# mbortolon97/6dgs

Hardware: AMD Instinct MI355X
Metric: poses/sec (higher is better)
Workload: dtype f32

## Files before the change

### 6dgs_amd/_lib.py

```python
from __future__ import annotations

import ctypes as C
import os

_HERE = os.path.dirname(os.path.abspath(__file__))
LIB_PATH = os.path.join(_HERE, "csrc", "lib6dgs_hip.so")
if os.environ.get("SIXDGS_LIB"):
    LIB_PATH = os.path.abspath(os.environ["SIXDGS_LIB"])

vp = C.c_void_p
i64 = C.c_int64
i32 = C.c_int
sz = C.c_size_t


PROFILE_SLOTS = 128
ABI_VERSION = 10


class Profile(C.Structure):
    _fields_ = [("count", i32), ("start", vp * PROFILE_SLOTS), ("stop", vp * PROFILE_SLOTS),
                ("flops", C.c_double * PROFILE_SLOTS), ("bytes", C.c_double * PROFILE_SLOTS)]


# ... 5 lines not shown
    "sixdgs_abi_version": (i32, []),
    "sixdgs_error_string": (C.c_char_p, [i32]),
    "sixdgs_mask_degraded": (i32, [vp, i64, i32, vp, vp]),
    "sixdgs_sym_eig_3x3": (i32, [vp, i64, vp, vp, vp]),
    "sixdgs_normals_knn": (i32, [vp, i64, vp, i64, i32, vp, vp, vp]),
    "sixdgs_normals_knn_grid_workspace_bytes": (sz, [i64]),
    "sixdgs_normals_knn_grid": (i32, [vp, i64, vp, i64, i32, vp, vp, vp, sz, vp]),
    "sixdgs_emit_quadricell_count": (i32, [vp, vp, i32, vp, vp, i64, vp, i32, i32, vp, vp, vp, vp]),
    "sixdgs_emit_quadricell_write": (i32, [vp, vp, i32, vp, vp, vp, i32, i32, vp, i64, vp, i32, i32, vp, vp, vp, vp, vp, vp]),
    "sixdgs_quadricell_cell_counts": (i32, [vp, i64, i32, vp, vp, vp, vp]),
    "sixdgs_quadricell_centers": (i32, [vp, i64, i32, i32, vp, vp, vp, vp]),
    "sixdgs_isocell_distribution": (i32, [i32, i32, vp, C.POINTER(i64), vp]),
    "sixdgs_rotate_isocell": (i32, [vp, i64, vp, i64, vp, vp]),
    "sixdgs_emit_isocell": (i32, [vp, vp, i32, vp, vp, vp, i32, i32, vp, i64, vp, vp, i64, vp, vp, vp, vp, vp]),
    "sixdgs_eval_sh_color": (i32, [vp, i32, vp, i64, i32, vp, vp]),
    "sixdgs_splat_views_workspace_bytes": (sz, [i64, i32, i32, i32]),
    "sixdgs_splat_views": (i32, [vp, vp, i32, vp, vp, i32, i32, i64, vp, i32, i32, i32, i32, C.c_float, C.c_float, vp, vp, vp, vp, sz, vp]),
    "sixdgs_raster_views_workspace_bytes": (sz, [i64, i32, i32, i32, i64]),
    "sixdgs_raster_views": (i32, [vp, vp, i32, vp, vp, i32, vp, vp, i32, i32, i64, vp, i32, i32, i32, C.c_float, vp, vp, vp, i32, vp, i64, vp, vp, sz,
                                  vp, C.POINTER(Profile)]),
    "sixdgs_raster_views_backward_workspace_bytes": (sz, [i64, i32, i32, i32, i64]),
    "sixdgs_raster_views_backward": (i32, [vp, vp, i32, vp, vp, i32, vp, vp, i32, i32, i64, vp, i32, i32, i32, C.c_float, vp, vp, i64, vp, sz,
                                           vp, vp, vp, vp, vp, vp, vp, vp, sz, vp, C.POINTER(Profile)]),
    "sixdgs_photometric_loss_workspace_bytes": (sz, [i32, i32, i32, i32]),
    "sixdgs_photometric_loss": (i32, [vp, i32, vp, i32, i32, i32, i32, i32, C.c_float, vp, vp, vp, vp, vp, sz, vp, C.POINTER(Profile)]),
    "sixdgs_pose_compose": (i32, [vp, vp, i32, vp, vp]),
    "sixdgs_pose_step": (i32, [vp, vp, vp, vp, i64, i32, i32, i32, C.c_float, C.c_float, C.c_float, C.c_float] + [vp] * 10 + [vp]),
    "sixdgs_refine_poses_workspace_bytes": (sz, [i64, i32, i32, i32, i64]),
    "sixdgs_refine_poses": (i32, [vp, vp, i32, vp, vp, i32, vp, vp, i32, i32, i64, vp, i32, i32, i32, C.c_float, vp, vp, i32, i32, C.c_float,
                                  i32, C.c_float, C.c_float, C.c_float, C.c_float, i64] + [vp] * 7 + [vp, sz, vp]),
    "sixdgs_target_pyramid": (i32, [vp, i32, i32, i32, i32, i32, vp, i32, vp, vp, vp]),
    "sixdgs_pose_rebase": (i32, [vp, vp, i32, vp, vp]),
    "sixdgs_refine_poses_levels_workspace_bytes": (sz, [i64, i32, i32, vp, vp, vp]),
    "sixdgs_refine_poses_levels": (i32, [vp, vp, i32, vp, vp, i32, vp, vp, i32, i32, i64, vp, i32, C.c_float, vp, C.c_float, i32] + [vp] * 7
                                   + [C.c_float, C.c_float, C.c_float] + [vp] * 8 + [vp, sz, vp]),
    "sixdgs_gaussian_adam": (i32, [i64, i32, i32] + [vp] * 6 + [vp] * 6 + [vp, vp, vp, C.c_float, C.c_float, C.c_float, vp, i64, vp, vp]),
    "sixdgs_opacity_reset": (i32, [vp, i64, i32, vp, vp, C.c_float, vp]),
    "sixdgs_fit_scene_workspace_bytes": (sz, [i64, i32, i32, i32, i32, i64]),
    "sixdgs_fit_scene": (i32, [vp, vp, i32, vp, vp, i32, vp, vp, i32, i64, vp, i32, i32, i32, C.c_float, vp, vp, i32, i32, C.c_float, i32, i32,
                               vp, vp, vp, vp, i32, C.c_float, C.c_float, C.c_float, C.c_float, i64] + [vp] * 5 + [vp, sz, vp]),
    "sixdgs_densify_stats": (i32, [i64, i32, i32, i32, i64, vp, sz, vp, sz, vp, vp, vp, vp, vp, vp, vp]),
    "sixdgs_densify_workspace_bytes": (sz, [i64]),
    "sixdgs_densify": (i32, [i64, i32] + [vp] * 6 + [i32, i32] + [vp] * 6 + [C.c_float] * 4 + [i32, i32, i64] + [vp] * 8 + [vp, vp, vp, sz, vp]),
    "sixdgs_knn_workspace_bytes": (sz, [i64]),
    "sixdgs_knn_mean_dist2": (i32, [i64, vp, vp, vp, sz, vp]),
    "sixdgs_fit_scene_steps_workspace_bytes": (sz, [i64, i32, i32, i32, i32, i64]),
    "sixdgs_fit_scene_steps": (i32, [vp, vp, i32, vp, vp, i32, vp, vp, i32, i64, vp, i32, i32, i32, C.c_float, vp, vp, i32, i32, C.c_float, i32, i32,
                                     vp, vp, vp, vp, vp, vp, i32, i32, C.c_float, C.c_float, C.c_float, C.c_float, i64] + [vp] * 5 + [vp] * 3
                               + [vp, sz, vp]),
    "sixdgs_packed_weights_floats": (sz, []),
    "sixdgs_pack_weights": (i32, [vp] * 13 + [C.POINTER(ScorerWeights), vp]),
    "sixdgs_ray_encode": (i32, [vp, vp, vp, i64, vp, vp]),
    "sixdgs_ray_keys_workspace_bytes": (sz, [i64, i64]),
    "sixdgs_ray_keys": (i32, [vp, vp, vp, i64, C.POINTER(ScorerWeights), vp, vp, vp, sz, vp]),
    "sixdgs_ray_keys_ex": (i32, [vp, vp, vp, i64, C.POINTER(ScorerWeights), vp, vp, vp, vp, vp, vp, sz, vp, C.POINTER(Profile), i32]),
    "sixdgs_key_planes_f16_bytes": (sz, [i64]),
    "sixdgs_split_planes_f16": (i32, [vp, i64, i64, vp, vp, vp]),
    "sixdgs_score_pass1": (i32, [vp, vp, vp, i32, vp, vp, vp, i64, i32, vp, vp, sz, vp, C.POINTER(Profile), i32]),
    "sixdgs_score_pass2": (i32, [vp, vp, i32, i32, i64, i32, vp, vp, vp, vp, sz, vp, i32]),
    "sixdgs_score_backward_workspace_bytes": (sz, [i32]),
    "sixdgs_score_backward": (i32, [vp, vp, i32, vp, i64, vp, vp, vp, vp, vp, sz, vp]),
    "sixdgs_score_backward_split_workspace_bytes": (sz, [i32, i64, i32]),
    "sixdgs_score_backward_split": (i32, [vp, vp, i32, vp, i64, vp, vp, vp, vp, i32, vp, sz, vp]),
    "sixdgs_score_topk_ex": (i32, [vp, vp, vp, i32, vp, vp, vp, i64, i32, vp, vp, vp, vp, vp, sz, vp, C.POINTER(Profile), i32]),
    "sixdgs_score_select_workspace_bytes": (sz, [i64, i32, i32, i32]),
    "sixdgs_score_select": (i32, [vp, vp, vp, i32, vp, vp, vp, i64, vp, vp, i64, i32, i32, vp, vp, vp, vp, sz, vp, C.POINTER(Profile)]),
    "sixdgs_tok_attention": (i32, [vp, i64, i32, i32, i32, vp, i64, vp]),
    "sixdgs_im2col": (i32, [vp, i64, i64, i64, i64, i32, i32, i32, i32, i32, i32, vp, vp]),
    "sixdgs_u8_to_planar": (i32, [vp, i32, i64, vp, vp, vp]),
    "sixdgs_image_prep": (i32, [vp, i32, i32, i32, vp, i32, i32, i32, i32, i32, vp, vp, vp, vp]),
    "sixdgs_tok_pack_bytes": (sz, [i32, i32]),
    "sixdgs_tok_pack": (i32, [vp, i32, i32, i64, vp, vp, vp]),
    "sixdgs_tok_linear": (i32, [vp, i64, i32, i64, i32, vp, vp, C.c_float, vp, vp, vp, i32, i32, vp, i64, vp, vp, i64, vp]),
    "sixdgs_key_planes_norm_max": (i32, [vp, vp, i64, vp, vp]),
    "sixdgs_select_workspace_bytes": (sz, [i64, i32, i32, i32]),
    "sixdgs_select_candidates_workspace_bytes": (sz, [i64, i32, i32, i32]),
    "sixdgs_select_begin": (i32, [vp, vp, vp, i32, vp, vp, i64, i64, vp, vp, vp, sz, vp]),
    "sixdgs_select_sweep_plan": (i32, [vp, i32, vp, vp, i32]),
    "sixdgs_select_sweep": (i32, [vp, vp, vp, i32, vp, vp, i64, vp, vp, vp, i64, vp, vp, sz, vp, C.POINTER(Profile)]),
    "sixdgs_select_candidates": (i32, [vp, i64, i64, vp, vp, vp, i32, vp, vp, vp, i32, i32, vp, vp, vp, sz, vp]),
    "sixdgs_select_rescore": (i32, [vp, vp, i32, vp, vp, i32, vp, vp, vp, vp, i64, i32, i32, i32, vp, vp, vp, vp, sz, vp]),
    "sixdgs_select_sample_stats": (i32, [vp, vp, vp, i32, vp, vp, i64, vp, vp, sz, vp]),
    "sixdgs_select_prepare": (i32, [vp, vp, i32, i64, i64, vp, vp, vp]),
    "sixdgs_select_topk_u": (i32, [vp, i64, i64, vp, i32, i32, vp, vp, sz, vp]),
    "sixdgs_linear_splitk_workspace_bytes": (sz, [i64, i32, i32]),
    "sixdgs_linear_splitk": (i32, [vp, i64, i32, i64, vp, i64, vp, i32, i32, vp, i64, i32, vp, sz, vp, i32]),
    "sixdgs_linear_ex": (i32, [vp, i64, i32, i64, vp, i64, vp, i32, i32, vp, i64, vp, i32]),
    "sixdgs_profile_collect": (i32, [C.POINTER(Profile), C.POINTER(C.c_double), C.POINTER(C.c_double), C.POINTER(C.c_double),
                                    C.POINTER(i32)]),
    "sixdgs_linear": (i32, [vp, i64, i32, i64, vp, i64, vp, i32, i32, vp, i64, vp]),
    "sixdgs_q_proj": (i32, [vp, vp, i32, C.POINTER(ScorerWeights), vp, vp]),
    "sixdgs_score_topk_workspace_bytes": (sz, [i64, i32, i32]),
    "sixdgs_score_topk_workspace_bytes_ex": (sz, [i64, i32, i32, i32, i32]),
    "sixdgs_score_topk": (i32, [vp, vp, i32, vp, i64, i32, vp, vp, vp, vp, vp, sz, vp]),
    "sixdgs_topk_workspace_bytes": (sz, [i64, i32, i32]),
    "sixdgs_topk": (i32, [vp, i64, i32, i32, vp, vp, vp, sz, vp]),
    "sixdgs_distance_target_workspace_bytes": (sz, [i64]),
    "sixdgs_distance_target": (i32, [vp, vp, i64, vp, i32, vp, vp, vp, sz, vp]),
    "sixdgs_solve_pose": (i32, [vp, vp, i64, vp, vp, i32, vp, vp, i32, vp, vp, vp, vp, vp, vp, vp]),
    "sixdgs_solve_pose_consensus_workspace_bytes": (sz, [i32, i32]),
    "sixdgs_solve_pose_consensus": (i32, [vp, vp, i64, vp, vp, i32, vp, vp, i32, C.c_float, i32] + [vp] * 10 + [vp, sz, vp]),
}

_lib = None


def load():
    global _lib
    if _lib is not None:
        return _lib
    import torch

    if not os.path.exists(LIB_PATH):
        raise RuntimeError(
            f"6dgs_amd: {LIB_PATH} is missing -- build it with `python -m 6dgs_amd.build` / __graft_entry__.build(); "
            "there is no CPU fallback for the product path")
    try:
        lib = C.CDLL(LIB_PATH)
    except OSError as e:
        raise RuntimeError(f"6dgs_amd: cannot load {LIB_PATH}: {e}") from e
    for name, (res, args) in SIGNATURES.items():
        try:
            fn = getattr(lib, name)
        except AttributeError as e:
            raise RuntimeError(f"6dgs_amd: {LIB_PATH} does not export {name}") from e
        fn.restype = res
        fn.argtypes = args
    if lib.sixdgs_abi_version() != ABI_VERSION:
        raise RuntimeError(f"6dgs_amd: ABI version mismatch (library {lib.sixdgs_abi_version()}, binding {ABI_VERSION})")
    _lib = lib
    return lib


def check(status: int, what: str = ""):
    if status != 0:
        msg = load().sixdgs_error_string(int(status)).decode()
        raise RuntimeError(f"6dgs_amd: {what or 'call'} failed: {msg} (status {status})")
```

### 6dgs_amd/build.py

```python
from __future__ import annotations

import os
import subprocess
import sys

HERE = os.path.dirname(os.path.abspath(__file__))
CSRC = os.path.join(HERE, "csrc")
LIB = os.path.join(CSRC, "lib6dgs_hip.so")
HOSTCHECK = os.path.join(CSRC, "libsixdgs_hostcheck.so")
SOURCES = ["geometry.hip", "gemm.hip", "dense.hip", "score.hip", "score_bwd.hip", "pose.hip", "pose_consensus.hip", "vit.hip", "splat.hip", "raster.hip", "photometric.hip", "refine.hip", "fit.hip", "densify.hip", "knn.hip", "pyramid.hip"]
HEADERS = ["common.h", "device_math.h", "gemm_kernel.h", "dense.h", os.path.join("..", "..", "include", "sixdgs.h"), "dense_layout.h", "sweep_plan.h", "sweep_layout.h", "pose_step.h", "adam_step.h", "render_pass.h", "densify_rules.h", "knn_rules.h", "pyramid_rules.h"]
HIPCC = os.environ.get("HIPCC", "/opt/rocm/bin/hipcc")
FLAGS = ["--offload-arch=gfx950", "-O3", "-std=c++17", "-fPIC", "-ffp-contract=off", "-Wall", "-Wno-unused-function"]
FLAGS += os.environ.get("SIXDGS_EXTRA_FLAGS", "").split()


def _stale(target, deps):
    if not os.path.exists(target):
        return True
    t = os.path.getmtime(target)
    return any(os.path.getmtime(d) > t for d in deps)


def build(force: bool = False, verbose: bool = False) -> str:
    deps = [os.path.join(CSRC, s) for s in SOURCES + HEADERS]
    if force or _stale(LIB, deps):
        objs = []
        procs = []
        for s in SOURCES:
            o = os.path.join(CSRC, s.replace(".hip", ".o"))
            objs.append(o)
            cmd = [HIPCC, *FLAGS, "-c", os.path.join(CSRC, s), "-o", o]
            if verbose:
                print(" ".join(cmd))
            procs.append((cmd, subprocess.Popen(cmd, stdout=subprocess.PIPE, stderr=subprocess.STDOUT, text=True)))
        for cmd, p in procs:
            out, _ = p.communicate()
            if p.returncode != 0:
                sys.stderr.write(out)
                raise RuntimeError("hipcc failed: " + " ".join(cmd))
            if verbose and out.strip():
                print(out)
        cmd = [HIPCC, "--offload-arch=gfx950", "-shared", "-fPIC", *objs, "-o", LIB]
        subprocess.check_call(cmd)
    return LIB


def build_hostcheck(force: bool = False) -> str:
    src = os.path.join(CSRC, "hostcheck.cpp")
    deps = [src, os.path.join(CSRC, "device_math.h"), os.path.join(CSRC, "dense_layout.h"), os.path.join(CSRC, "sweep_plan.h"),
            os.path.join(CSRC, "sweep_layout.h"), os.path.join(CSRC, "pose_step.h"), os.path.join(CSRC, "adam_step.h"), os.path.join(CSRC, "densify_rules.h"),
            os.path.join(CSRC, "knn_rules.h"), os.path.join(CSRC, "pyramid_rules.h")]
    if force or _stale(HOSTCHECK, deps):
        cmd = [HIPCC, "-x", "hip", "--offload-arch=gfx950", "-O2", "-std=c++17", "-fPIC", "-ffp-contract=off", "-shared", src,
               "-o", HOSTCHECK]
        subprocess.check_call(cmd)
    return HOSTCHECK


if __name__ == "__main__":
    print(build(force="--force" in sys.argv, verbose=True))
    print(build_hostcheck(force="--force" in sys.argv))
```

### 6dgs_amd/csrc/hostcheck.cpp

```cpp
#include <stdlib.h>

#include "device_math.h"
#include "sweep_plan.h"
#include "dense_layout.h"
#include "sweep_layout.h"
#include "pose_step.h"
#include "adam_step.h"
#include "densify_rules.h"
#include "knn_rules.h"
#include "pyramid_rules.h"

#include <algorithm>
#include <vector>
using namespace sdg;

extern "C" {

void hc_mask_degraded(const float* scale, long long n, int P, unsigned char* mask) {
  for (long long i = 0; i < n; ++i) {
    float side;
    mask[i] = total_rings(scale[3 * i], scale[3 * i + 1], scale[3 * i + 2], (float)P, &side) < (long long)P;
  }
}

long long hc_quadricell_centers(const float* scale, long long E, int P, int res, float* points, long long* eid) {
  long long C = 0;
  float* table = (float*)malloc(sizeof(float) * res);
  for (long long e = 0; e < E; ++e) {
    float a = scale[3 * e], b = scale[3 * e + 1], c = scale[3 * e + 2], side;
    long long rings = total_rings(a, b, c, (float)P, &side);
    for (long long ring = 0; ring < rings; ++ring) {
      Ring rg = ring_params(a, b, c, side, (float)rings, (float)ring);
      int npts = ring_cells(rg);
      if (!npts) continue;
      if (points) {
        double acc = 0.0;
        table[0] = 0.f;
        for (int j = 0; j < res - 1; ++j) { acc += (double)ring_table_increment(rg, j); table[j + 1] = (float)acc; }
        float last = table[res - 1];
        for (int j = 0; j < res; ++j) table[j] = kTwoPi * (table[j] / last);
        for (int j = 0; j < npts; ++j) {
          int pick = ring_table_pick(table, res, (float)j * rg.dtheta);
          V3 p = ring_point(rg, table[pick]);
          points[3 * (C + j)] = p.x; points[3 * (C + j) + 1] = p.y; points[3 * (C + j) + 2] = p.z;
          eid[C + j] = e;
        }
      }
      C += npts;
    }
  }
  free(table);
  return C;
}

long long hc_emit_rays(const float* points, const long long* eid, long long C, const float* normals, const float* centers,
                       const float* rot4, float* ori, float* dir, long long* mid) {
  long long r = 0;
  for (long long i = 0; i < C; ++i) {
    long long e = eid[i];
    float R[9];
    quat_to_rotmat(rot4 + 4 * e, R);
    V3 pw = rotate(R, v3(points[3 * i], points[3 * i + 1], points[3 * i + 2]));
    if (!hemisphere_keep(normals[3 * e], pw)) continue;
    V3 d = normalize_eps(pw);
    ori[3 * r] = pw.x + centers[3 * e]; ori[3 * r + 1] = pw.y + centers[3 * e + 1]; ori[3 * r + 2] = pw.z + centers[3 * e + 2];
    dir[3 * r] = d.x; dir[3 * r + 1] = d.y; dir[3 * r + 2] = d.z;
    mid[r++] = e;
  }
  return r;
}

void hc_sym_eig(const float* mats, long long n, float* vals, float* vecs) {
  for (long long i = 0; i < n; ++i) sym_eig_3x3(mats + 9 * i, vals + 3 * i, vecs ? vecs + 9 * i : nullptr);
}

void hc_normals_from_knn(const float* cloud, const long long* knn, long long nq, int k, float* normals) {
  float* nb = (float*)malloc(sizeof(float) * 3 * k);
  for (long long q = 0; q < nq; ++q) {
    for (int j = 0; j < k; ++j)
      for (int c = 0; c < 3; ++c) nb[3 * j + c] = cloud[3 * knn[q * k + j] + c];
    V3 n = normal_from_neighbours(nb, k);
    normals[3 * q] = n.x; normals[3 * q + 1] = n.y; normals[3 * q + 2] = n.z;
  }
  free(nb);
}

long long hc_isocell_dirs(int target, int n0, float* dirs) {
  int n = isocell_rings(target, n0);
// ... 167 lines not shown
void hc_knn_pair_d2(long long n, const float* q, const float* p, float* out) {
  for (long long i = 0; i < n; ++i) out[i] = kn::pair_d2(q[3 * i], q[3 * i + 1], q[3 * i + 2], p[3 * i], p[3 * i + 1], p[3 * i + 2]);
}
int hc_knn_boxed(long long n, const float* xyz, int box, float* mean_d2, int* visited) {
  if (n < 4 || box < 1) return -1;
  float lo[3], hi[3];
  for (int a = 0; a < 3; ++a) lo[a] = INFINITY, hi[a] = -INFINITY;
  for (long long i = 0; i < n; ++i)
    for (int a = 0; a < 3; ++a) {
      lo[a] = fminf(lo[a], xyz[3 * i + a]);
      hi[a] = fmaxf(hi[a], xyz[3 * i + a]);
    }
  std::vector<unsigned> code(n);
  std::vector<long long> order(n);
  for (long long i = 0; i < n; ++i) {
    code[i] = kn::morton(xyz + 3 * i, lo, hi);
    order[i] = i;
  }
  std::stable_sort(order.begin(), order.end(), [&](long long a, long long b) { return code[a] < code[b]; });
  const long long nb = (n + box - 1) / box;
  std::vector<float> s(3 * n), blo(3 * nb, INFINITY), bhi(3 * nb, -INFINITY);
  for (long long k = 0; k < n; ++k)
    for (int a = 0; a < 3; ++a) {
      const float c = s[3 * k + a] = xyz[3 * order[k] + a];
      blo[3 * (k / box) + a] = fminf(blo[3 * (k / box) + a], c);
      bhi[3 * (k / box) + a] = fmaxf(bhi[3 * (k / box) + a], c);
    }
  for (long long k = 0; k < n; ++k) {
    const float qx = s[3 * k], qy = s[3 * k + 1], qz = s[3 * k + 2];
    float b0 = INFINITY, b1 = INFINITY, b2 = INFINITY;
    const long long own = k / box;
    int walked = 0;
    for (long long step = 0; step < nb; ++step)
      for (int side = 0; side < (step ? 2 : 1); ++side) {
        const long long c = side ? own + step : own - step;
        if (c < 0 || c >= nb) continue;
        if (step && kn::box_d2(qx, qy, qz, &blo[3 * c], &bhi[3 * c]) >= b2) continue;
        ++walked;
        const long long end = std::min(n, (c + 1) * box);
        for (long long j = c * box; j < end; ++j)
          if (j != k) kn::insert3(kn::pair_d2(qx, qy, qz, s[3 * j], s[3 * j + 1], s[3 * j + 2]), b0, b1, b2);
      }
    mean_d2[order[k]] = kn::mean3(b0, b1, b2);
    if (visited) visited[order[k]] = walked;
  }
  return 0;
}
int hc_pyr_max_levels() { return pyr::kMaxLevels; }
int hc_pyr_max_downscale() { return pyr::kMaxDownscale; }
void hc_pyr_geometry(int W, int H, int d, const float* k4, int* geo4, float* k_out4) {
  const pyr::Level g = pyr::level_geometry(W, H, d);
  geo4[0] = g.w; geo4[1] = g.h; geo4[2] = g.ox; geo4[3] = g.oy;
  pyr::level_intrinsics(k4, d, g.ox, g.oy, k_out4);
}
int hc_pyr_target(const unsigned char* images, int views, int H, int W, int C, int composite, const float* background, int d, float* out) {
  if (d < 1 || d > pyr::kMaxDownscale || (C != 3 && C != 4) || (composite && C != 4)) return -1;
  const pyr::Level g = pyr::level_geometry(W, H, d);
  if (g.w < 1 || g.h < 1) return -1;
  float bg255[3] = {0.f, 0.f, 0.f};
  if (composite)
    for (int c = 0; c < 3; ++c) bg255[c] = pyr::background_term(background[c]);
  for (int v = 0; v < views; ++v)
    for (int y = 0; y < g.h; ++y)
      for (int x = 0; x < g.w; ++x)
        for (int c = 0; c < 3; ++c) {
          unsigned S = 0u, S2 = 0u;
          for (int j = 0; j < d; ++j)
            for (int i = 0; i < d; ++i) {
              const unsigned char* q = images + (((size_t)v * H + (size_t)(g.oy + y * d + j)) * W + (size_t)(g.ox + x * d + i)) * C;
              if (composite) {
                S += (unsigned)q[c] * (unsigned)q[3];
                S2 += 255u - (unsigned)q[3];
              } else {
                S += (unsigned)q[c];
              }
            }
          out[(((size_t)v * g.h + y) * g.w + x) * 3 + c] = composite ? pyr::value_composite(S, S2, bg255[c], d) : pyr::value_plain(S, d);
        }
  return 0;
}
void hc_pyr_keep_input(const float* best_loss_last, const float* loss_input, long long n, int* keep) {
  for (long long i = 0; i < n; ++i) keep[i] = pyr::keep_input(best_loss_last[i], loss_input[i]) ? 1 : 0;
}
int hc_dl_const(int which) {
  const int v[] = {dl::kSlabB, dl::kPRow, dl::kGran, dl::kGranSlab, dl::kChunkRun};
  return which >= 0 && which < 5 ? v[which] : -1;
}

}
```

### 6dgs_amd/csrc/score.hip

```cpp
#include <stdlib.h>

#include <cstdlib>
#include <cstdio>
#include "gemm_kernel.h"
#include "sweep_plan.h"
#include "sweep_layout.h"

using namespace sdg;

namespace {

constexpr int kT = SIXDGS_MAX_TOKENS;
constexpr float kSqrtD = 19.595917942265423f;

struct LogitsArgs {
  const float* q;
  const int* n_tok;
  const float* key;
  float* logits;
  float* partial;
  int64_t r, ldl;
  int tiles_per_group, n_tiles, n_groups;
  int b0;
};

template <int MMA>
__global__ void __launch_bounds__(256, 2) k_logits(LogitsArgs A) {
  __shared__ __attribute__((aligned(16))) char smem[TileSmem<MMA>::kBytes];
  __shared__ float part[2][128][2];
  const int bl = blockIdx.y;
  const int b = A.b0 + bl;
  const unsigned w = xcd_remap(blockIdx.x, gridDim.x);
  const int grp = (int)(w >> 1), m_tile = (int)(w & 1u);
  const int M = A.n_tok[b];
  const int row0 = m_tile * 128;
  float* pout = A.partial + (((int64_t)bl * A.n_groups + grp) * kT + row0) * 2;
  const int tid = threadIdx.x, lane = tid & 63, wave = tid >> 6;
  const int wm = wave >> 1, wn = wave & 1;
  float m_run = -INFINITY, s_run = 0.f;
  if (row0 < M) {
    GemmOperands g = {A.q + (int64_t)b * kT * SIXDGS_D, nullptr, A.key, SIXDGS_D, 0, SIXDGS_D, M, A.r, SIXDGS_D, SIXDGS_D};
    float* lg = A.logits + (int64_t)bl * kT * A.ldl;
    const int t_begin = grp * A.tiles_per_group;
    const int t_end = min(t_begin + A.tiles_per_group, A.n_tiles);
    for (int tile = t_begin; tile < t_end; ++tile) {
      const int64_t col0 = (int64_t)tile * kBN;
      f32x16 acc[2][2];
      gemm_tile<MMA>(g, row0, col0, smem, acc);
      const int64_t c0 = col0 + acc_col(wn, 0, lane), c1 = col0 + acc_col(wn, 1, lane);
      const bool v0 = c0 < A.r, v1 = c1 < A.r;
#pragma unroll
      for (int tm = 0; tm < 2; ++tm)
#pragma unroll
        for (int r = 0; r < 16; ++r) {
          const int row = row0 + acc_row(wm, tm, r, lane);
          const float l0 = acc[tm][0][r] / kSqrtD, l1 = acc[tm][1][r] / kSqrtD;
          if (row < M) {
            if (v0) lg[(int64_t)row * A.ldl + c0] = l0;
            if (v1) lg[(int64_t)row * A.ldl + c1] = l1;
          }
          float mx = fmaxf(v0 ? l0 : -INFINITY, v1 ? l1 : -INFINITY);
#pragma unroll
          for (int o = 16; o > 0; o >>= 1) mx = fmaxf(mx, __shfl_xor(mx, o, 64));
          float sm = 0.f;
          if (mx > -INFINITY) sm = (v0 ? expf(l0 - mx) : 0.f) + (v1 ? expf(l1 - mx) : 0.f);
#pragma unroll
          for (int o = 16; o > 0; o >>= 1) sm += __shfl_xor(sm, o, 64);
          if ((lane & 31) == 0) {
            const int lr = acc_row(wm, tm, r, lane);
            part[wn][lr][0] = mx;
            part[wn][lr][1] = sm;
          }
        }
      __syncthreads();
      if (tid < 128) {
#pragma unroll
        for (int h = 0; h < 2; ++h) {
          const float mt = part[h][tid][0], st = part[h][tid][1];
          if (mt > -INFINITY) {
            const float mn = fmaxf(m_run, mt);
            s_run = s_run * expf(m_run - mn) + st * expf(mt - mn);
            m_run = mn;
          }
        }
      }
    }
  }
  if (tid < 128) {
    pout[2 * tid] = m_run;
// ... 688 lines not shown
          if (!ragged) {
#pragma unroll
            for (int tn = 0; tn < 4; ++tn)
#pragma unroll
              for (int r = 0; r < 16; ++r) sum[r & 3] += __expf(acc[tm][tn][r] - mn);
          } else {
            int ray0 = wn * 128 + 4 * (lane >> 5);
            asm volatile("" : "+v"(ray0));
#pragma unroll
            for (int tn = 0; tn < 4; ++tn)
#pragma unroll
              for (int r = 0; r < 16; ++r)
                sum[r & 3] += (ray0 + tn * 32 + 8 * (r >> 2) + (r & 3) <= lim_cur) ? __expf(acc[tm][tn][r] - mn) : 0.f;
          }
          s_run[tm] = s_run[tm] * __expf(m_run[tm] - mn) + ((sum[0] + sum[1]) + (sum[2] + sum[3]));
          m_run[tm] = mn;
        }
      }
      kcur = knext;
      lim_cur = lim_next;
    }
    if constexpr (PIPE) {
      if (active) {
#pragma unroll
        for (int rb = 4; rb < sw::kRayBlocks; ++rb) {
#pragma unroll
          for (int k = 0; k < 8; ++k) sweep_epi_exp(E, acc16, zs16, ct16, lane_p, wn, rb, k >> 2, k & 3);
          sweep_epi_fold_a(E, lane_p);
          sweep_epi_fold_b(E, lane_p, rb);
          sweep_epi_fold_c(E, lane_p, rb);
        }
        sweep_epi_store(E, lane_p, 1);
      }
    }
    asm volatile("s_waitcnt vmcnt(0)" ::: "memory");
  }
  __syncthreads();
  float(*part)[256][2] = reinterpret_cast<float(*)[256][2]>(lds);
  if (S16) {
    int lm = lane;
    if (PERS) asm volatile("" : "+v"(lm));
#pragma unroll
    for (int tb = 0; tb < sw::kTokBlocks; ++tb) {
      float z = zs16[tb];
      z += __builtin_bit_cast(float, __builtin_amdgcn_ds_swizzle(__builtin_bit_cast(int, z), 0x401F));
      if (sw::part_writes(lm)) {
        float* pp = part[sw::part_row(wn, lm)][wm * 64 + sw::acc_token(lm, tb)];
        pp[0] = 0.f;
        pp[1] = z;
      }
    }
  } else {
#pragma unroll
  for (int tm = 0; tm < 2; ++tm) {
    float* pp = part[wn * 2 + (lane >> 5)][wm * 64 + tm * 32 + (lane & 31)];
    if (OUT == kOutUB) {
      pp[0] = 0.f;
      pp[1] = (zs[tm][0].x + zs[tm][0].y) + (zs[tm][1].x + zs[tm][1].y);
    } else {
      pp[0] = m_run[tm];
      pp[1] = s_run[tm];
    }
  }
  }
  __syncthreads();
  if (tid < 256) {
    float m = -INFINITY, sres = 0.f;
#pragma unroll
    for (int h = 0; h < 4; ++h) {
      const float mt = part[h][tid][0], st2 = part[h][tid][1];
      if (mt > -INFINITY) {
        const float mn = fmaxf(m, mt);
        sres = sres * __expf(m - mn) + st2 * __expf(mt - mn);
        m = mn;
      }
    }
    pout[2 * tid] = m;
    pout[2 * tid + 1] = sres;
  }
  if (PERS) __syncthreads();
  } while (PERS && (grp += A.n_sets) < A.n_groups);
}

__global__ void __launch_bounds__(256) k_split_tiles_f16(const float* __restrict__ src, int64_t rows, int64_t ld, char* __restrict__ dst,
                                                         float* __restrict__ inv_scale) {
  __shared__ float wmax[4];
  const int64_t row0 = (int64_t)blockIdx.x * 128;
  const int n = (int)min((int64_t)128, rows - row0);
  const float* base = src + row0 * ld;
  float m = 0.f;
  for (int i = threadIdx.x; i < n * 96; i += 256) {
    const int row = i / 96;
    const float4 v = *reinterpret_cast<const float4*>(base + (int64_t)row * ld + (i - row * 96) * 4);
    m = fmaxf(m, fmaxf(fmaxf(fabsf(v.x), fabsf(v.y)), fmaxf(fabsf(v.z), fabsf(v.w))));
  }
  m = sdg_wave_max(m);
  if (sdg_lane() == 0) wmax[sdg_wave()] = m;
  __syncthreads();
  m = fmaxf(fmaxf(wmax[0], wmax[1]), fmaxf(wmax[2], wmax[3]));
  int sh = 0;
  if (m > 0.f && m < INFINITY) {
    int e;
    frexpf(m, &e);
    sh = 14 - e;
    sh = sh > 100 ? 100 : (sh < -100 ? -100 : sh);
  }
  const float sc = ldexpf(1.f, sh);
  if (threadIdx.x == 0) inv_scale[blockIdx.x] = ldexpf(1.f, -sh);
  for (int i = threadIdx.x; i < n * 48; i += 256) {
    const int row = i / 48, k8 = i - row * 48;
    const float* sp = base + (int64_t)row * ld + k8 * 8;
    const float4 lo = *reinterpret_cast<const float4*>(sp);
    const float4 hi = *reinterpret_cast<const float4*>(sp + 4);
    const float x[8] = {lo.x * sc, lo.y * sc, lo.z * sc, lo.w * sc, hi.x * sc, hi.y * sc, hi.z * sc, hi.w * sc};
    f16x8 h, l;
#pragma unroll
    for (int e = 0; e < 8; ++e) {
      const _Float16 hh = (_Float16)x[e];
      h[e] = hh;
      l[e] = (_Float16)(x[e] - (float)hh);
    }
    char* d = dst + (row0 + row) * kRowF + (k8 >> 2) * kSlabF + (k8 & 3) * 16;
    *reinterpret_cast<f16x8*>(d) = h;
    *reinterpret_cast<f16x8*>(d + 64) = l;
  }
}

__global__ void __launch_bounds__(256) k_split_q_tiles_f16(const float* __restrict__ q, const int* __restrict__ n_tok, char* __restrict__ dst,
                                                           float* __restrict__ inv_scale) {
  __shared__ float wmax[4];
  const int bl = blockIdx.x >> 1, half = blockIdx.x & 1;
  const int n = min(128, max(0, n_tok[bl] - 128 * half));
  const float* base = q + ((int64_t)bl * kT + 128 * half) * SIXDGS_D;
  float m = 0.f;
  for (int i = threadIdx.x; i < n * 96; i += 256) {
    const float4 v = *reinterpret_cast<const float4*>(base + (int64_t)i * 4);
    m = fmaxf(m, fmaxf(fmaxf(fabsf(v.x), fabsf(v.y)), fmaxf(fabsf(v.z), fabsf(v.w))));
  }
  m = sdg_wave_max(m);
  if (sdg_lane() == 0) wmax[sdg_wave()] = m;
  __syncthreads();
  m = fmaxf(fmaxf(wmax[0], wmax[1]), fmaxf(wmax[2], wmax[3]));
  int sh = 0;
  if (m > 0.f && m < INFINITY) {
    int e;
    frexpf(m, &e);
    sh = 14 - e;
    sh = sh > 100 ? 100 : (sh < -100 ? -100 : sh);
  }
  const float sc = ldexpf(1.f, sh);
  if (threadIdx.x == 0) inv_scale[blockIdx.x] = ldexpf(1.f, -sh);
  char* const drow = dst + ((int64_t)bl * kT + 128 * half) * kRowF;
  for (int i = threadIdx.x; i < 128 * 48; i += 256) {
    const int row = i / 48, k8 = i - row * 48;
    f16x8 h, l;
    if (row < n) {
      const float* sp = base + (int64_t)row * SIXDGS_D + k8 * 8;
      const float4 lo = *reinterpret_cast<const float4*>(sp);
      const float4 hi = *reinterpret_cast<const float4*>(sp + 4);
      const float x[8] = {lo.x * sc, lo.y * sc, lo.z * sc, lo.w * sc, hi.x * sc, hi.y * sc, hi.z * sc, hi.w * sc};
#pragma unroll
      for (int e = 0; e < 8; ++e) {
        const _Float16 hh = (_Float16)x[e];
        h[e] = hh;
        l[e] = (_Float16)(x[e] - (float)hh);
      }
// ... 266 lines not shown
      if (w2 < wv) { og += sc[0][w2]; oe += sc[1][w2]; }
      tg += sc[0][w2];
      te += sc[1][w2];
    }
    __syncthreads();
    if (WRITE) {
      const unsigned long long below = (1ull << lane) - 1ull;
      if (gt) {
        const unsigned pos = base_g + run_g + og + __popcll(bg & below);
        if (pos < (unsigned)topk) { cand_key[(int64_t)b * topk + pos] = key; cand_idx[(int64_t)b * topk + pos] = i; }
      } else if (eq) {
        const unsigned re = base_e + run_e + oe + __popcll(be & below);
        if (re < st.remain) {
          const unsigned pos = n_greater + re;
          if (pos < (unsigned)topk) { cand_key[(int64_t)b * topk + pos] = key; cand_idx[(int64_t)b * topk + pos] = i; }
        }
      }
    }
    run_g += tg;
    run_e += te;
  }
  if (!WRITE && threadIdx.x == 0) {
    counts[((int64_t)b * gridDim.x + blockIdx.x) * 2] = run_g;
    counts[((int64_t)b * gridDim.x + blockIdx.x) * 2 + 1] = run_e;
  }
}

__global__ void __launch_bounds__(1024) k_topk_scan(const unsigned* __restrict__ counts, int nb, unsigned* __restrict__ offs, const int* __restrict__ only) {
  __shared__ unsigned sm[17];
  const int b = blockIdx.x;
  if (only != nullptr && only[b] == 0) return;
  for (int comp = 0; comp < 2; ++comp) {
    unsigned base = 0;
    for (int c0 = 0; c0 < nb; c0 += 1024) {
      const int i = c0 + threadIdx.x;
      const unsigned v = i < nb ? counts[((int64_t)b * nb + i) * 2 + comp] : 0u;
      unsigned tot;
      const unsigned ex = sdg_block_exclusive_scan<unsigned, 16>(v, sm, &tot);
      if (i < nb) offs[((int64_t)b * nb + i) * 2 + comp] = base + ex;
      base += tot;
    }
  }
}

__global__ void __launch_bounds__(1024) k_topk_sort(const unsigned* __restrict__ cand_key, const int64_t* __restrict__ cand_idx,
                                                     int topk, int k_eff, int64_t* __restrict__ idx, float* __restrict__ val, const int* __restrict__ only) {
  __shared__ unsigned sk[1024];
  __shared__ long long si[1024];
  const int b = blockIdx.x, t = threadIdx.x;
  if (only != nullptr && only[b] == 0) return;
  if (t < k_eff) { sk[t] = cand_key[(int64_t)b * topk + t]; si[t] = cand_idx[(int64_t)b * topk + t]; }
  else { sk[t] = 0u; si[t] = 0x7fffffffffffffffll; }
  __syncthreads();
  for (int size = 2; size <= 1024; size <<= 1)
    for (int strd = size >> 1; strd > 0; strd >>= 1) {
      const int p = t ^ strd;
      if (p > t) {
        const bool up = (t & size) == 0;
        const unsigned ka = sk[t], kb = sk[p];
        const long long ia = si[t], ib = si[p];
        const bool a_first = ka > kb || (ka == kb && ia < ib);
        if (up ? !a_first : a_first) { sk[t] = kb; sk[p] = ka; si[t] = ib; si[p] = ia; }
      }
      __syncthreads();
    }
  if (t < topk) {
    if (t < k_eff) { idx[(int64_t)b * topk + t] = si[t]; val[(int64_t)b * topk + t] = key_score(sk[t]); }
    else { idx[(int64_t)b * topk + t] = -1; val[(int64_t)b * topk + t] = NAN; }
  }
}

constexpr float kLog2e = 1.4426950408889634f;

__global__ void __launch_bounds__(kT) k_sel_prepare(const float* __restrict__ stats_s, const int* __restrict__ n_tok, int b0, float log2_frac,
                                                    float* __restrict__ ctok) {
  const int bl = blockIdx.x, t = threadIdx.x;
  const float m = stats_s[((int64_t)bl * kT + t) * 2], z = stats_s[((int64_t)bl * kT + t) * 2 + 1];
  const bool ok = t < n_tok[b0 + bl] && z > 0.f && m > -INFINITY && m < INFINITY;
  ctok[(int64_t)bl * kT + t] = ok ? -(m * kLog2e) - (log2f(z) + log2_frac) : -INFINITY;
}

__global__ void __launch_bounds__(256) k_split_q_slots(const float* __restrict__ q, const int* __restrict__ n_tok, const SweepSlots T, char* __restrict__ dst,
                                                       float* __restrict__ inv_scale, const float* __restrict__ ctok, float* __restrict__ ctok_slot,
                                                       int* __restrict__ slot_rows) {
  __shared__ float wmax[4];
  const int slot = blockIdx.x >> 2, w = blockIdx.x & 3;
  const int img = T.q_img[slot][w], lq = T.q_lq[slot][w];
  const int n = img < 0 ? 0 : min(64, max(0, n_tok[img] - 64 * lq));
  const float* base = q + ((int64_t)(img < 0 ? 0 : img) * kT + 64 * (lq < 0 ? 0 : lq)) * SIXDGS_D;
  float m = 0.f;
  for (int i = threadIdx.x; i < n * 96; i += 256) {
    const float4 v = *reinterpret_cast<const float4*>(base + (int64_t)i * 4);
    m = fmaxf(m, fmaxf(fmaxf(fabsf(v.x), fabsf(v.y)), fmaxf(fabsf(v.z), fabsf(v.w))));
  }
  m = sdg_wave_max(m);
  if (sdg_lane() == 0) wmax[sdg_wave()] = m;
  __syncthreads();
  m = fmaxf(fmaxf(wmax[0], wmax[1]), fmaxf(wmax[2], wmax[3]));
  int sh = 0;
  if (m > 0.f && m < INFINITY) {
    int e;
    frexpf(m, &e);
    sh = 14 - e;
    sh = sh > 100 ? 100 : (sh < -100 ? -100 : sh);
  }
  const float sc = ldexpf(1.f, sh);
  if (threadIdx.x == 0) inv_scale[blockIdx.x] = ldexpf(1.f, -sh);
  char* const drow = dst + ((int64_t)slot * kT + 64 * w) * kRowF;
  for (int i = threadIdx.x; i < 64 * 48; i += 256) {
    const int row = i / 48, k8 = i - row * 48;
    f16x8 h, l;
    if (row < n) {
      const float* sp = base + (int64_t)row * SIXDGS_D + k8 * 8;
      const float4 lo = *reinterpret_cast<const float4*>(sp);
      const float4 hi = *reinterpret_cast<const float4*>(sp + 4);
      const float x[8] = {lo.x * sc, lo.y * sc, lo.z * sc, lo.w * sc, hi.x * sc, hi.y * sc, hi.z * sc, hi.w * sc};
#pragma unroll
      for (int e = 0; e < 8; ++e) {
        const _Float16 hh = (_Float16)x[e];
        h[e] = hh;
        l[e] = (_Float16)(x[e] - (float)hh);
      }
    } else {
#pragma unroll
      for (int e = 0; e < 8; ++e) h[e] = l[e] = (_Float16)0.f;
    }
    char* d = drow + (int64_t)row * kRowF + (k8 >> 2) * kSlabF + (k8 & 3) * 16;
    *reinterpret_cast<f16x8*>(d) = h;
    *reinterpret_cast<f16x8*>(d + 64) = l;
  }
  if (ctok_slot != nullptr && threadIdx.x < 64) {
    const int t = threadIdx.x;
    ctok_slot[(int64_t)slot * kT + 64 * w + t] = t < n ? ctok[(int64_t)img * kT + 64 * lq + t] : -INFINITY;
  }
  if (w == 0 && threadIdx.x == 0) {
    int rows = 0;
    for (int x = 0; x < kSlotQuarters; ++x) {
      const int im = T.q_img[slot][x];
      const int nx = im < 0 ? 0 : min(64, max(0, n_tok[im] - 64 * T.q_lq[slot][x]));
      if (nx > 0) rows = 64 * x + nx;
    }
    slot_rows[slot] = rows;
  }
}

__global__ void __launch_bounds__(1024) k_merge_stats_slots(const float* __restrict__ partial, int n_groups, const SweepSlots T, float* __restrict__ stats,
                                                            float* __restrict__ gsum) {
  __shared__ float sm[16][64][2];
  const int k = blockIdx.x, y = blockIdx.y, tl = threadIdx.x & 63, j = threadIdx.x >> 6;
  const int img = T.img[k], sq = y < T.img_nq[k] ? T.img_q[k][y] : -1;
  float m = -INFINITY, s = 0.f;
  if (sq >= 0) {
    const float* p = partial + (int64_t)(sq >> 2) * n_groups * kT * 2;
    const int row = 64 * (sq & 3) + tl;
    for (int g = j; g < n_groups; g += 16) {
      const float mt = p[((int64_t)g * kT + row) * 2], st = p[((int64_t)g * kT + row) * 2 + 1];
      if (mt > -INFINITY) {
        const float mn = fmaxf(m, mt);
        s = s * expf(m - mn) + st * expf(mt - mn);
        m = mn;
      }
    }
  }
  sm[j][tl][0] = m;
  sm[j][tl][1] = s;
  __syncthreads();
  if (j == 0) {
    m = -INFINITY;
    s = 0.f;
#pragma unroll
    for (int qd = 0; qd < 16; ++qd) {
      const float mt = sm[qd][tl][0], st = sm[qd][tl][1];
      if (mt > -INFINITY) {
        const float mn = fmaxf(m, mt);
        s = s * expf(m - mn) + st * expf(mt - mn);
        m = mn;
      }
    }
    const int64_t o = (int64_t)img * kT + 64 * y + tl;
    if (gsum != nullptr) {
      gsum[o] += s;
    } else {
      stats[o * 2] = m;
      stats[o * 2 + 1] = s;
    }
  }
}

__global__ void __launch_bounds__(256) k_sel_finish_slots(const float* __restrict__ ub, int64_t stride, int64_t u_stride, const int* __restrict__ n_tok, const SweepSlots T,
                                                          int64_t R, float* __restrict__ U, float* __restrict__ tmax, int64_t tmax_stride) {
  const int k = blockIdx.y, img = T.img[k];
  const int nq_dev = (min(max(n_tok[img], 0), kT) + 63) >> 6;
  const int nq = min(nq_dev, (int)T.img_nq[k]);
  const int64_t i = ((int64_t)blockIdx.x * blockDim.x + threadIdx.x) * 4;
  float m = -INFINITY;
  if (i < R) {
    float4 a = {0.f, 0.f, 0.f, 0.f};
    const int64_t row[kSlotQuarters] = {T.img_q[k][0], T.img_q[k][1], T.img_q[k][2], T.img_q[k][3]};
#pragma unroll
    for (int y = 0; y < kSlotQuarters; ++y)
      if (y < nq) {
        const float4 v = *reinterpret_cast<const float4*>(ub + row[y] * stride + i);
        a.x += v.x; a.y += v.y; a.z += v.z; a.w += v.w;
      }
    *reinterpret_cast<float4*>(U + (int64_t)img * u_stride + i) = a;
    m = a.x;
    if (i + 1 < R) m = fmaxf(m, a.y);
    if (i + 2 < R) m = fmaxf(m, a.z);
// ... 752 lines not shown
  while (g > 256 && n_tiles_x / g < 16) g -= 256;
  if (g > n_tiles_x) g = n_tiles_x;
  return g;
}

int sibling_sync_mode() {
  static int mode = -1;
  if (mode < 0) {
    const char* e = getenv("SIXDGS_SIBLING_SYNC");
    mode = e ? atoi(e) : kSiblingSyncDefault;
  }
  return mode;
}
bool sweep_mfma16() {
  const char* e = getenv("SIXDGS_SWEEP_MFMA");
  return !(e && atoi(e) == 32);
}
bool sweep_epilogue_tile() {
  const char* e = getenv("SIXDGS_SWEEP_EPILOGUE");
  return e && e[0] == 't' && e[1] == 'i' && e[2] == 'l' && e[3] == 'e' && e[4] == 0;
}
int sibling_sync_cus() {
  static int cus = -1;
  if (cus < 0) {
    const bool on = sibling_sync_mode() != 0;
    int dev = 0;
    hipDeviceProp_t prop;
    cus = (on && hipGetDevice(&dev) == hipSuccess && hipGetDeviceProperties(&prop, dev) == hipSuccess && prop.multiProcessorCount > 0) ? prop.multiProcessorCount : 0;
  }
  return cus;
}

void select_q_planes(const float* q, int nb, const SelectWs& w, hipStream_t s) {
  hipLaunchKernelGGL(k_split_tiles_f16, dim3((unsigned)(2 * nb)), dim3(256), 0, s, q, (int64_t)nb * kT, (int64_t)SIXDGS_D, w.qplanes, w.qinv);
}
LogitsF16Args select_args(const int32_t* d_n_tok, int nb, const SelectWs& w, const void* planes, const float* scale, int64_t r) {
  LogitsF16Args V = {w.qplanes, d_n_tok, (const char*)planes, w.qinv, scale, nullptr, w.partial, r, w.p.stride, 0, 0, 0, 0, nb, nullptr, nullptr, 0};
  V.n_tiles = (int)sdg_cdiv(r, kBNX);
  V.n_groups = f16x_groups(r);
  V.tiles_per_group = (int)sdg_cdiv(V.n_tiles, V.n_groups);
  return V;
}
}

extern "C" {

size_t sixdgs_select_workspace_bytes(int64_t r, int batch, int topk, int max_candidates) {
  if (batch < 1) batch = 1;
  const SelectPlan p = select_plan(r, batch, topk, max_candidates);
  return p.topk_bytes + (size_t)batch * p.per_image;
}

size_t sixdgs_select_candidates_workspace_bytes(int64_t r, int batch, int topk, int max_candidates) {
  if (batch < 1) batch = 1;
  const SelectPlan p = select_plan(r, batch, topk, max_candidates, false);
  return p.topk_bytes + (size_t)batch * p.per_image;
}

static int sweep_slot_cap() {
  static const int cap = [] {
    const char* e = getenv("SIXDGS_SWEEP_MAX_IMAGES");
    const int v = e ? atoi(e) : kSweepMaxImages;
    if (e && v <= 0) fprintf(stderr, "6dgs_amd: SIXDGS_SWEEP_MAX_IMAGES=%s: launches of %d slots (the slot table's limit), a last one of up to %d -- not one launch per batch\n", e, kSweepMaxSlots * 2 / 3, kSweepMaxSlots * 2 / 3 + kSweepMaxSlots / 3);
    return v;
  }();
  return cap;
}

static bool prepass_one_term(int ) {
  static const int forced = [] { const char* e = getenv("SIXDGS_PREPASS_TERMS"); return e ? atoi(e) : 0; }();
  return forced == 1 || (forced != 3 && kPrepassOneTermDefault);
}

int sixdgs_select_sweep_plan(const int32_t* h_n_tok, int batch, int32_t* slots_per_launch, int32_t* images_per_launch, int max_launches) {
  if (batch < 0 || batch > 32767 || max_launches < 0 || (max_launches > 0 && (!slots_per_launch || !images_per_launch))) return SIXDGS_E_BADARG;
  const std::vector<SweepSlots> plan = sweep_pack(h_n_tok, batch, sweep_slot_cap());
  for (size_t l = 0; l < plan.size() && (int)l < max_launches; ++l) {
    slots_per_launch[l] = plan[l].n_slots;
    images_per_launch[l] = plan[l].n_images;
  }
  return (int)plan.size();
}

int sixdgs_select_sample_stats(const float* q, const int32_t* d_n_tok, const int32_t* h_n_tok, int batch, const void* sample_planes,
                               const float* d_sample_scale, int64_t r_sample, float* row_stats, void* ws, size_t ws_bytes, sixdgs_stream_t stream) {
  SDG_CHECK_ARG(batch >= 0 && batch <= 32767 && r_sample >= 1);
  if (batch == 0) return 0;
  SDG_CHECK_ARG(q && d_n_tok && sample_planes && d_sample_scale && row_stats && ws && ((uintptr_t)sample_planes % 16) == 0 &&
                ((uintptr_t)q % 16) == 0 && ((uintptr_t)ws % 256) == 0);
  hipStream_t s = sdg_stream(stream);
  SelectWs w;
  if (!select_ws(ws, ws_bytes, r_sample, batch, 1, 8, &w)) return SIXDGS_E_WORKSPACE;
  const int n_groups = f16x_groups(r_sample);
  for (const SweepSlots& T : sweep_pack(h_n_tok, batch, sweep_slot_cap())) {
    if (T.n_slots > 0) {
      hipLaunchKernelGGL(k_split_q_slots, dim3((unsigned)(4 * T.n_slots)), dim3(256), 0, s, q, d_n_tok, T, w.qplanes, w.qinv, (const float*)nullptr,
                         (float*)nullptr, w.slot_rows);
      LogitsF16Args V = select_args(w.slot_rows, T.n_slots, w, sample_planes, d_sample_scale, r_sample);
      V.q_quarter_scales = 1;
      static const int reserve_env = [] { const char* e = getenv("SIXDGS_PREPASS_RESERVE_CUS"); return e ? atoi(e) : -2; }();
      const int reserve = reserve_env != -2 ? reserve_env : (T.n_slots == 1 ? kPrepassReserveCusOneSlot : kPrepassReserveCus);
      const int cus = sibling_sync_cus();
      if (reserve >= 0 && cus > reserve && (cus - reserve) / T.n_slots >= 1) {
        V.n_sets = (cus - reserve) / T.n_slots < V.n_groups ? (cus - reserve) / T.n_slots : V.n_groups;
        V.sib_sync = nullptr;
        V.sib_extra = 0u;
        V.sib_period = kSibPeriod;
        if (prepass_one_term(T.n_slots)) hipLaunchKernelGGL((k_logits_f16x<kOneTerm, kOutStats, true>), dim3((unsigned)(V.n_sets * T.n_slots)), dim3(512), 0, s, V);
        else hipLaunchKernelGGL((k_logits_f16x<kAllTerms, kOutStats, true>), dim3((unsigned)(V.n_sets * T.n_slots)), dim3(512), 0, s, V);
      } else {
        if (prepass_one_term(T.n_slots)) hipLaunchKernelGGL((k_logits_f16x<kOneTerm, kOutStats>), dim3((unsigned)(V.n_groups * T.n_slots)), dim3(512), 0, s, V);
        else hipLaunchKernelGGL((k_logits_f16x<kAllTerms, kOutStats>), dim3((unsigned)(V.n_groups * T.n_slots)), dim3(512), 0, s, V);
      }
    }
    hipLaunchKernelGGL(k_merge_stats_slots, dim3((unsigned)T.n_images, 4), dim3(1024), 0, s, w.partial, n_groups, T, row_stats, (float*)nullptr);
  }
  SDG_LAUNCH_OK();
  return 0;
}

int sixdgs_select_prepare(const float* row_stats, const int32_t* d_n_tok, int batch, int64_t r_sample, int64_t r_total, float* ctok, float* gsum,
                          sixdgs_stream_t stream) {
  SDG_CHECK_ARG(batch >= 0 && r_sample >= 1 && r_total >= r_sample);
  if (batch == 0) return 0;
  SDG_CHECK_ARG(row_stats && d_n_tok && ctok && gsum);
  hipStream_t s = sdg_stream(stream);
  hipLaunchKernelGGL(k_sel_prepare, dim3((unsigned)batch), dim3(kT), 0, s, row_stats, d_n_tok, 0, log2f((float)((double)r_total / (double)r_sample)), ctok);
  hipError_t e = hipMemsetAsync(gsum, 0, (size_t)batch * kT * sizeof(float), s);
  if (e != hipSuccess) return (int)e;
  SDG_LAUNCH_OK();
  return 0;
}

int sixdgs_select_begin(const float* q, const int32_t* d_n_tok, const int32_t* h_n_tok, int batch, const void* sample_planes, const float* d_sample_scale,
                        int64_t r_sample, int64_t r_total, float* ctok, float* gsum, void* ws, size_t ws_bytes, sixdgs_stream_t stream) {
  SDG_CHECK_ARG(batch >= 0 && r_sample >= 1 && r_total >= r_sample);
  if (batch == 0) return 0;
  SDG_CHECK_ARG(ws && ((uintptr_t)ws % 256) == 0);
  SelectWs w;
  if (!select_ws(ws, ws_bytes, r_sample, batch, 1, 8, &w)) return SIXDGS_E_WORKSPACE;
  const int st = sixdgs_select_sample_stats(q, d_n_tok, h_n_tok, batch, sample_planes, d_sample_scale, r_sample, w.stats, ws, ws_bytes, stream);
  if (st) return st;
  return sixdgs_select_prepare(w.stats, d_n_tok, batch, r_sample, r_total, ctok, gsum, stream);
}

int sixdgs_select_sweep(const float* q, const int32_t* d_n_tok, const int32_t* h_n_tok, int batch, const void* key_planes,
                        const float* d_key_scale, int64_t r, const float* ctok, float* gsum, float* u, int64_t u_stride, float* u_tile_max,
                        void* ws, size_t ws_bytes, sixdgs_stream_t stream, sixdgs_profile* prof) {
  SDG_CHECK_ARG(batch >= 0 && batch <= 32767 && r >= 1 && u_stride >= sdg_cdiv(r, 256) * 256 && (u_stride % 4) == 0 && (!u_tile_max || (u_stride % 256) == 0));
  if (batch == 0) return 0;
  SDG_CHECK_ARG(q && d_n_tok && key_planes && d_key_scale && ctok && gsum && u && ws && ((uintptr_t)key_planes % 16) == 0 &&
                ((uintptr_t)q % 16) == 0 && ((uintptr_t)u % 16) == 0 && ((uintptr_t)ws % 256) == 0);
  hipStream_t s = sdg_stream(stream);
  SelectWs w;
  if (!select_ws(ws, ws_bytes, r, batch, 1, 8, &w)) return SIXDGS_E_WORKSPACE;
  const int n_groups = f16x_groups(r);
  for (const SweepSlots& T : sweep_pack(h_n_tok, batch, sweep_slot_cap())) {
    const int ns = T.n_slots;
    double tok = 0.0;
    for (int k = 0; k < T.n_images; ++k) tok += h_n_tok ? (double)(h_n_tok[T.img[k]] < 0 ? 0 : (h_n_tok[T.img[k]] > kT ? kT : h_n_tok[T.img[k]])) : (double)kT;
    if (ns > 0) {
      hipLaunchKernelGGL(k_split_q_slots, dim3((unsigned)(4 * ns)), dim3(256), 0, s, q, d_n_tok, T, w.qplanes, w.qinv, ctok, w.ctok_slot, w.slot_rows);
      LogitsF16Args V = select_args(w.slot_rows, ns, w, key_planes, d_key_scale, r);
      V.q_quarter_scales = 1;
      V.ctok = w.ctok_slot;
      V.ub = w.ub;
      V.ub_stride = w.p.stride;
      unsigned grid = (unsigned)(V.n_groups * ns);
      const int cus = sibling_sync_cus();
      if (cus > 0 && ns >= 2 && cus / ns >= 1 && (cus % ns) * 16 <= cus && w.p.topk_bytes >= (size_t)(cus / ns) * sizeof(unsigned)) {
        V.n_sets = cus / ns < V.n_groups ? cus / ns : V.n_groups;
        V.sib_sync = sibling_sync_mode() == 2 ? nullptr : reinterpret_cast<unsigned*>(w.topk_ws);
        V.sib_extra = sibling_sync_mode() == 3 ? 1u : 0u;
        V.sib_period = kSibPeriod;
        if (V.sib_sync && hipMemsetAsync(V.sib_sync, 0, (size_t)V.n_sets * sizeof(unsigned), s) != hipSuccess) return (int)hipGetLastError();
        grid = (unsigned)(V.n_sets * ns);
      }
      SdgProfileScope scope(prof, s, 2.0 * tok * SIXDGS_D * (double)r, (double)r * (kRowF + T.n_images * 16.0));
      auto kern = sweep_mfma16() ? (sweep_epilogue_tile() ? (V.n_sets > 0 ? k_logits_f16x<kAllTerms, kOutUB, true, kMfma16Tile> : k_logits_f16x<kAllTerms, kOutUB, false, kMfma16Tile>)
                                                          : (V.n_sets > 0 ? k_logits_f16x<kAllTerms, kOutUB, true, kMfma16> : k_logits_f16x<kAllTerms, kOutUB, false, kMfma16>))
                                 : (V.n_sets > 0 ? k_logits_f16x<kAllTerms, kOutUB, true> : k_logits_f16x<kAllTerms, kOutUB, false>);
      hipLaunchKernelGGL(kern, dim3(grid), dim3(512), 0, s, V);
    }
    hipLaunchKernelGGL(k_merge_stats_slots, dim3((unsigned)T.n_images, 4), dim3(1024), 0, s, w.partial, n_groups, T, (float*)nullptr, gsum);
    hipLaunchKernelGGL(k_sel_finish_slots, dim3((unsigned)sdg_cdiv(r, 1024), (unsigned)T.n_images), dim3(256), 0, s, w.ub, w.p.stride, u_stride, d_n_tok, T, r, u,
                       u_tile_max, u_stride / 256);
  }
  SDG_LAUNCH_OK();
  return 0;
}

int sixdgs_key_planes_norm_max(const void* planes, const float* d_scale, int64_t rows, float* d_norm_max, sixdgs_stream_t stream) {
  SDG_CHECK_ARG(rows >= 0);
  if (rows == 0) return 0;
  SDG_CHECK_ARG(planes && d_scale && d_norm_max && ((uintptr_t)planes % 16) == 0);
  const int64_t blocks = sdg_cdiv(rows, 4);
  hipLaunchKernelGGL(k_plane_norm_max, dim3((unsigned)(blocks < 8192 ? blocks : 8192)), dim3(256), 0, sdg_stream(stream), (const char*)planes, d_scale,
                     rows, reinterpret_cast<unsigned*>(d_norm_max));
  SDG_LAUNCH_OK();
  return 0;
}

int sixdgs_select_topk_u(const float* u, int64_t u_stride, int64_t r, const float* u_tile_max, int batch, int topk, float* val, void* ws,
                         size_t ws_bytes, sixdgs_stream_t stream) {
  SDG_CHECK_ARG(batch >= 0 && r >= 1 && u_stride >= r && topk >= 1 && topk <= 1024);
  if (batch == 0) return 0;
  SDG_CHECK_ARG(u && val && ws && ((uintptr_t)ws % 256) == 0);
  SelectWs w;
  if (!select_ws(ws, ws_bytes, r, batch, topk, 8, &w, false)) return SIXDGS_E_WORKSPACE;
  const int64_t nt = sdg_cdiv(r, 256);
  if (u_tile_max && nt >= 2 * (int64_t)topk) return run_topk(u_tile_max, u_stride / 256, nt, batch, topk, w.idxU, val, w.topk_ws, sdg_stream(stream));
  return run_topk(u, u_stride, r, batch, topk, w.idxU, val, w.topk_ws, sdg_stream(stream));
}

int sixdgs_select_candidates(const float* u, int64_t u_stride, int64_t r, const float* u_tile_max, const float* q, const int32_t* d_n_tok, int batch,
                             const float* gsum, const float* d_key_norm_max, const float* d_uk, int topk, int max_candidates, int64_t* cand,
                             int32_t* d_count, void* ws, size_t ws_bytes, sixdgs_stream_t stream) {
  SDG_CHECK_ARG(batch >= 0 && r >= 1 && u_stride >= r && topk >= 1 && topk <= 1024 && max_candidates >= topk && (max_candidates % 8) == 0);
  if (batch == 0) return 0;
  SDG_CHECK_ARG(u && q && d_n_tok && gsum && d_key_norm_max && cand && d_count && ws && ((uintptr_t)ws % 256) == 0 && ((uintptr_t)q % 16) == 0);
  hipStream_t s = sdg_stream(stream);
  SelectWs w;
  if (!select_ws(ws, ws_bytes, r, batch, topk, max_candidates, &w, false)) return SIXDGS_E_WORKSPACE;
  const int k_eff = (int)(r < topk ? r : topk);
  const dim3 cg((unsigned)w.p.nbc, (unsigned)batch);
  const int64_t nt = sdg_cdiv(r, 256);
  const bool tiles = !d_uk && u_tile_max && nt >= 2 * (int64_t)topk;
  const int* none = nullptr;
  if (d_uk) {
    hipLaunchKernelGGL(k_sel_bounds, dim3((unsigned)batch), dim3(kT), 0, s, gsum, d_n_tok, d_uk, q, d_key_norm_max, 1, 1, w.info, none);
  } else if (!tiles) {
    int st = run_topk(u, u_stride, r, batch, topk, w.idxU, w.valU, w.topk_ws, s);
    if (st) return st;
    hipLaunchKernelGGL(k_sel_bounds, dim3((unsigned)batch), dim3(kT), 0, s, gsum, d_n_tok, w.valU, q, d_key_norm_max, topk, k_eff, w.info, none);
  } else {
    int* need = w.total + batch;
    int st = run_topk(u_tile_max, u_stride / 256, nt, batch, topk, w.idxU, w.valU, w.topk_ws, s);
    if (st) return st;
    hipLaunchKernelGGL(k_sel_bounds, dim3((unsigned)batch), dim3(kT), 0, s, gsum, d_n_tok, w.valU, q, d_key_norm_max, topk, topk, w.info, none);
    hipLaunchKernelGGL(k_sel_candidates<false>, cg, dim3(256), 0, s, u, u_stride, r, w.info, w.p.span, w.counts, w.offs, cand, max_candidates, none, u_tile_max);
    hipLaunchKernelGGL(k_sel_scan, dim3((unsigned)batch), dim3(1024), 0, s, w.counts, w.p.nbc, w.offs, w.total);
    hipLaunchKernelGGL(k_sel_need_exact, dim3((unsigned)sdg_cdiv(batch, 64)), dim3(64), 0, s, w.total, w.info, batch, max_candidates, need);
    st = run_topk(u, u_stride, r, batch, topk, w.idxU, w.valU, w.topk_ws, s, need);
    if (st) return st;
    hipLaunchKernelGGL(k_sel_bounds, dim3((unsigned)batch), dim3(kT), 0, s, gsum, d_n_tok, w.valU, q, d_key_norm_max, topk, k_eff, w.info, need);
    hipLaunchKernelGGL(k_sel_candidates<false>, cg, dim3(256), 0, s, u, u_stride, r, w.info, w.p.span, w.counts, w.offs, cand, max_candidates, need, u_tile_max);
    hipLaunchKernelGGL(k_sel_scan, dim3((unsigned)batch), dim3(1024), 0, s, w.counts, w.p.nbc, w.offs, w.total);
    hipLaunchKernelGGL(k_sel_candidates<true>, cg, dim3(256), 0, s, u, u_stride, r, w.info, w.p.span, w.counts, w.offs, cand, max_candidates, none, u_tile_max);
  }
  if (!tiles) {
    hipLaunchKernelGGL(k_sel_candidates<false>, cg, dim3(256), 0, s, u, u_stride, r, w.info, w.p.span, w.counts, w.offs, cand, max_candidates, none, u_tile_max);
    hipLaunchKernelGGL(k_sel_scan, dim3((unsigned)batch), dim3(1024), 0, s, w.counts, w.p.nbc, w.offs, w.total);
    hipLaunchKernelGGL(k_sel_candidates<true>, cg, dim3(256), 0, s, u, u_stride, r, w.info, w.p.span, w.counts, w.offs, cand, max_candidates, none, u_tile_max);
  }
  hipLaunchKernelGGL(k_sel_count, dim3((unsigned)sdg_cdiv(batch, 64)), dim3(64), 0, s, w.total, w.info, batch, d_count);
  SDG_LAUNCH_OK();
  return 0;
}

int sixdgs_select_rescore(const float* q, const int32_t* d_n_tok, int batch, const void* planes, const float* d_scale, int compact,
                          const float* ctok, const float* gsum, const int64_t* cand, const int32_t* d_count, int64_t r, int topk,
                          int max_candidates, int allow_fewer, int64_t* idx, float* val, int32_t* d_status, void* ws, size_t ws_bytes,
                          sixdgs_stream_t stream) {
  SDG_CHECK_ARG(batch >= 0 && r >= 1 && topk >= 1 && topk <= 1024 && max_candidates >= topk && (max_candidates % 8) == 0);
  if (batch == 0) return 0;
  SDG_CHECK_ARG(q && d_n_tok && planes && d_scale && ctok && gsum && cand && d_count && idx && val && d_status && ws &&
                ((uintptr_t)planes % 16) == 0 && ((uintptr_t)q % 16) == 0 && ((uintptr_t)ws % 256) == 0);
  hipStream_t s = sdg_stream(stream);
  const int cmax = max_candidates;
  SelectWs w;
  if (!select_ws(ws, ws_bytes, cmax, batch, topk, cmax, &w, false)) return SIXDGS_E_WORKSPACE;
  const int k_eff = (int)(r < topk ? r : topk);
  select_q_planes(q, batch, w, s);
  hipLaunchKernelGGL(k_sel_rescore, dim3((unsigned)(cmax / 8), (unsigned)batch), dim3(kT), 0, s, w.qplanes, w.qinv, (const char*)planes, d_scale,
                     d_n_tok, 0, ctok, gsum, cand, d_count, cmax, compact, w.cscore);
  const int st = run_topk(w.cscore, cmax, cmax, batch, topk, w.lidx, w.lval, w.topk_ws, s);
  if (st) return st;
  hipLaunchKernelGGL(k_sel_emit, dim3((unsigned)batch), dim3(1024), 0, s, w.lidx, w.lval, cand, d_count, cmax, topk, k_eff, allow_fewer, idx, val, d_status);
  SDG_LAUNCH_OK();
  return 0;
}

size_t sixdgs_score_select_workspace_bytes(int64_t r, int batch, int topk, int max_candidates) {
  if (batch < 1) batch = 1;
  const size_t stride = (size_t)sdg_cdiv(r > 0 ? r : 1, 256) * 256;
  return sdg_align(sixdgs_select_workspace_bytes(r, batch, topk, max_candidates)) +
         (size_t)batch * (2 * sdg_align(kT * sizeof(float)) + sdg_align(stride * sizeof(float)) + sdg_align(stride / 256 * sizeof(float)) +
                          sdg_align((size_t)max_candidates * sizeof(int64_t)) + 256);
}

int sixdgs_score_select(const float* q, const int32_t* d_n_tok, const int32_t* h_n_tok, int batch, const void* key_planes,
                        const float* d_key_scale, const float* d_key_norm_max, int64_t r, const void* sample_planes, const float* d_sample_scale,
                        int64_t r_sample, int topk, int max_candidates, int64_t* idx, float* val, int32_t* d_status, void* ws, size_t ws_bytes,
                        sixdgs_stream_t stream, sixdgs_profile* prof) {
  SDG_CHECK_ARG(r >= 1 && r_sample >= 1 && r_sample <= r && batch >= 0 && topk >= 1 && topk <= 1024 && max_candidates >= topk &&
                max_candidates <= (1 << 20) && (max_candidates % 8) == 0);
  if (batch == 0) return 0;
  SDG_CHECK_ARG(q && d_n_tok && d_key_norm_max && idx && val && d_status && ws && ((uintptr_t)ws % 256) == 0);
  int64_t bg = batch > 4096 ? 4096 : batch;
  while (bg >= 1 && sixdgs_score_select_workspace_bytes(r, (int)bg, topk, max_candidates) > ws_bytes) --bg;
  if (bg < 1) return SIXDGS_E_WORKSPACE;
  bg = sdg_cdiv(batch, sdg_cdiv(batch, bg));
  const size_t stride = (size_t)sdg_cdiv(r, 256) * 256;
  const size_t stage = sdg_align(sixdgs_select_workspace_bytes(r, (int)bg, topk, max_candidates));
  char* base = (char*)ws + stage;
  float* ctok = (float*)base;                        base += (size_t)bg * sdg_align(kT * sizeof(float));
  float* gsum = (float*)base;                        base += (size_t)bg * sdg_align(kT * sizeof(float));
  float* u = (float*)base;                           base += (size_t)bg * sdg_align(stride * sizeof(float));
  float* utm = (float*)base;                         base += (size_t)bg * sdg_align(stride / 256 * sizeof(float));
  int64_t* cand = (int64_t*)base;                    base += (size_t)bg * sdg_align((size_t)max_candidates * sizeof(int64_t));
  int32_t* count = (int32_t*)base;
  for (int b0 = 0; b0 < batch; b0 += (int)bg) {
    const int nb = (int)((batch - b0) < bg ? (batch - b0) : bg);
    const float* qg = q + (int64_t)b0 * kT * SIXDGS_D;
    const int32_t* ng = d_n_tok + b0;
    int st = sixdgs_select_begin(qg, ng, h_n_tok ? h_n_tok + b0 : nullptr, nb, sample_planes, d_sample_scale, r_sample, r, ctok, gsum, ws, stage, stream);
    if (st) return st;
    st = sixdgs_select_sweep(qg, ng, h_n_tok ? h_n_tok + b0 : nullptr, nb, key_planes, d_key_scale, r, ctok, gsum, u, (int64_t)stride, utm, ws, stage,
                             stream, prof);
    if (st) return st;
    st = sixdgs_select_candidates(u, (int64_t)stride, r, utm, qg, ng, nb, gsum, d_key_norm_max, nullptr, topk, max_candidates, cand, count, ws, stage, stream);
    if (st) return st;
    st = sixdgs_select_rescore(qg, ng, nb, key_planes, d_key_scale, 0, ctok, gsum, cand, count, r, topk, max_candidates, 0,
                               idx + (int64_t)b0 * topk, val + (int64_t)b0 * topk, d_status + b0, ws, stage, stream);
    if (st) return st;
  }
  return 0;
}

}
```

### 6dgs_amd/distributed.py

```python
from __future__ import annotations

import datetime
import os
from typing import Callable, Optional, Tuple

import torch
import torch.distributed as dist

_SCENE_FIELDS = ("_xyz", "_scaling", "_rotation", "_features_dc", "_features_rest", "_opacity")


_single_rank_group = False
_long_group = None
_long_group_timeout_s = None


def init_from_env(backend: Optional[str] = None, set_device: bool = True) -> Tuple[int, int, int]:
    global _single_rank_group
    rank = int(os.environ.get("RANK", "0"))
    world = int(os.environ.get("WORLD_SIZE", "1"))
    local = int(os.environ.get("LOCAL_RANK", str(rank)))
    single = world == 1 and os.environ.get("SIXDGS_DIST_SINGLE") == "1"
    if (world > 1 or single) and not dist.is_initialized():
        os.environ.setdefault("MASTER_ADDR", "127.0.0.1")
# ... 252 lines not shown
    bufs = [torch.empty_like(t) for _ in range(dist.get_world_size())]
    dist.all_gather(bufs, t)
    return [float(b.item()) for b in bufs]


def _collective_device(t: torch.Tensor) -> torch.Tensor:
    return t.cpu() if (t.is_cuda and dist.get_backend() == "gloo") else t


def merge_row_stats(stats: torch.Tensor, group=None) -> torch.Tensor:
    if not is_dist():
        return stats
    dev = stats.device
    m = _collective_device(stats[..., 0].contiguous())
    sl = _collective_device(stats[..., 1].contiguous())
    mg = m.clone()
    dist.all_reduce(mg, op=dist.ReduceOp.MAX, group=group)
    scale = torch.where(torch.isinf(m) & (m < 0), torch.zeros_like(m), torch.exp(m - mg))
    sg = sl * scale
    dist.all_reduce(sg, op=dist.ReduceOp.SUM, group=group)
    return torch.stack([mg, sg], dim=-1).to(dev)


def merge_topk(idx_local: torch.Tensor, val: torch.Tensor, ray_offset: int, k: int, group=None):
    gidx = torch.where(idx_local >= 0, idx_local + int(ray_offset), idx_local)
    if is_dist() and group is not False:
        world = dist.get_world_size(group)
        dev = idx_local.device
        gi, gv = _collective_device(gidx.contiguous()), _collective_device(val.contiguous())
        bi = [torch.empty_like(gi) for _ in range(world)]
        bv = [torch.empty_like(gv) for _ in range(world)]
        dist.all_gather(bi, gi, group=group)
        dist.all_gather(bv, gv, group=group)
        gidx, val = torch.cat(bi, dim=1).to(dev), torch.cat(bv, dim=1).to(dev)
    pad = gidx < 0
    key = torch.where(pad, torch.full_like(val, -float("inf")), val)
    big = torch.iinfo(torch.int64).max
    order = torch.argsort(torch.where(pad, torch.full_like(gidx, big), gidx), dim=1, stable=True)
    key, gidx, val = key.gather(1, order), gidx.gather(1, order), val.gather(1, order)
    order = torch.argsort(key, dim=1, descending=True, stable=True)[:, :k]
    return gidx.gather(1, order), val.gather(1, order)


def score_topk_ray_sharded(q: torch.Tensor, n_tok: torch.Tensor, key: Optional[torch.Tensor], ray_offset: int, topk: int = 100,
                           key_planes: Optional[torch.Tensor] = None, key_scale: Optional[torch.Tensor] = None, want_scores: bool = False,
                           workspace: Optional[torch.Tensor] = None, group=None):
    from . import ops

    r_local = key.shape[0] if key is not None else key_planes.shape[0]
    b = q.shape[0]
    if workspace is None:
        workspace = torch.empty(ops.score_topk_workspace_bytes(r_local, b, topk), dtype=torch.uint8, device=q.device)
    local = ops.score_pass1(q, n_tok, key, workspace, topk, key_planes=key_planes, key_scale=key_scale)
    glob = merge_row_stats(local, group)
    idx, val, scores = ops.score_pass2(glob, n_tok, r_local, workspace, topk, used_planes=key_planes is not None, want_scores=want_scores)
    gidx, gval = merge_topk(idx, val, ray_offset, topk, group)
    return gidx, gval, scores


def kth_largest_of_union(val_local: torch.Tensor, k: int, group=None) -> torch.Tensor:
    v = val_local
    if is_dist() and group is not False:
        world = dist.get_world_size(group)
        c = _collective_device(v.contiguous())
        bufs = [torch.empty_like(c) for _ in range(world)]
        dist.all_gather(bufs, c, group=group)
        v = torch.cat(bufs, dim=1).to(val_local.device)
    v = torch.where(torch.isnan(v), torch.full_like(v, -float("inf")), v)
    return torch.sort(v, dim=1, descending=True).values[:, k - 1].contiguous()


def _all_reduce(t: torch.Tensor, op, group=None) -> torch.Tensor:
    if not is_dist():
        return t
    c = _collective_device(t.contiguous())
    dist.all_reduce(c, op=op, group=group)
    if c is not t:
        t.copy_(c.to(t.device))
    return t


def score_select_ray_sharded(q: torch.Tensor, n_tok: torch.Tensor, key_planes: torch.Tensor, key_scale: torch.Tensor, sample_planes: torch.Tensor,
                             sample_scale: torch.Tensor, ray_offset: int, r_total: int, r_sample_total: int, topk: int = 100,
                             max_candidates: Optional[int] = None, n_tok_host=None, profile=None, group=None, key_norm: Optional[torch.Tensor] = None):
    from . import ops

    r_local = key_planes.shape[0]
    cmax = ops.SELECT_MAX_CANDIDATES if max_candidates is None else int(max_candidates)
    with ops.arena_scope():
        ss = ops.SelectStream(q, n_tok, r_local, topk, cmax, n_tok_host)
        stats = merge_row_stats(ss.sample_stats(sample_planes, sample_scale), group)
        ss.prepare(stats, r_sample_total, r_total)
        if key_norm is not None:
            ss.key_norm.copy_(key_norm)
        ss.sweep(key_planes, key_scale, 0, profile, update_norm=key_norm is None)
        _all_reduce(ss.gsum, dist.ReduceOp.SUM, group)
        _all_reduce(ss.key_norm, dist.ReduceOp.MAX, group)
        uk = kth_largest_of_union(ss.topk_u(exact=True), min(topk, r_total), group)
        cand, count = ss.candidates(uk=uk)
        idx, val, status = ss.rescore(key_planes, key_scale, cand, count, compact=False, allow_fewer=True)
        st = status.to(torch.int64)
        bad = _all_reduce((st < 0).to(torch.int64), dist.ReduceOp.MAX, group) if is_dist() else (st < 0).to(torch.int64)
        tot = _all_reduce(st.clamp(min=0), dist.ReduceOp.SUM, group) if is_dist() else st.clamp(min=0)
    gidx, gval = merge_topk(idx, val, ray_offset, topk, group)
    out_status = torch.where(bad > 0, torch.full_like(tot, -1), tot).tolist()
    for b, v in enumerate(out_status):
        if v < 0:
            gidx[b], gval[b] = -1, float("nan")
    return gidx, gval, out_status


def gather_selected_rays(gidx: torch.Tensor, ori_local: torch.Tensor, dir_local: torch.Tensor, ray_offset: int, group=None):
    r_local = ori_local.shape[0]
    loc = gidx - int(ray_offset)
    mine = (gidx >= 0) & (loc >= 0) & (loc < r_local)
    safe = torch.where(mine, loc, torch.zeros_like(loc))
    if r_local == 0:
        both = torch.zeros(*gidx.shape, 6, dtype=ori_local.dtype, device=ori_local.device)
    else:
        both = torch.cat([ori_local[safe], dir_local[safe]], dim=-1) * mine[..., None].to(ori_local.dtype)
    if is_dist() and group is not False:
        _all_reduce(both, dist.ReduceOp.SUM, group)
    return both[..., :3].contiguous(), both[..., 3:].contiguous()
```

### 6dgs_amd/identification_module.py

```python
from __future__ import annotations

from typing import List, Optional, Sequence

import torch

from . import ops
from .backbone import BackboneWrapper, BatchedTokens
from .camera_direction_network import CameraDirectionPredictor


def _lib_ray_keys_ws(r: int, max_chunk: int = ops.RAY_KEYS_CHUNK) -> int:
    from . import _lib
    return int(_lib.load().sixdgs_ray_keys_workspace_bytes(int(r), int(max_chunk)))


class RayPreprocessor(torch.nn.Module):

    def __init__(self, viewpe=8, pospe=8, rgbpe=6, featureC=128, fea_output=128):
        super().__init__()
        self.in_mlpC = 2 * viewpe * 3 + 3 + 2 * pospe * 3 + 3 + 2 * rgbpe * 3 + 3
        self.mlp = torch.nn.Sequential(torch.nn.Linear(self.in_mlpC, featureC), torch.nn.ReLU(inplace=True),
                                       torch.nn.Linear(featureC, featureC), torch.nn.ReLU(inplace=True))
        self.mlp2 = torch.nn.Sequential(torch.nn.Linear(featureC + self.in_mlpC, featureC), torch.nn.ReLU(inplace=True),
                                        torch.nn.Linear(featureC, fea_output))
# ... 18 lines not shown

    def __init__(self, n_tokens: int, n_rays: int, builder=None):
        self.shape = torch.Size((n_tokens, n_rays))
        self._builder = builder

    def materialize(self) -> torch.Tensor:
        if self._builder is None:
            raise RuntimeError("attention map not retained")
        return self._builder()


class IdentificationModule(torch.nn.Module):
    def __init__(self, backbone_type: str = "dino", camera_up_output_augmentation=None,
                 target_rays_dirs: Optional[torch.Tensor] = None, augmentation_channels: int = 10,
                 backbone: Optional[torch.nn.Module] = None):
        super().__init__()
        if camera_up_output_augmentation not in (None, 0, "NONE") and getattr(camera_up_output_augmentation, "name", "NONE") != "NONE":
            raise NotImplementedError("camera-up output augmentations are not on the accelerated path "
                                      "(reference default is NONE, identification_module.py:11,35-36)")
        self.backbone_wrapper = BackboneWrapper(backbone_type=backbone_type, backbone=backbone)
        nf = self.backbone_wrapper.img_num_features
        self.ray_preprocessor = RayPreprocessor(featureC=512, fea_output=nf)
        self.camera_up_out_augmentation = None
        self.camera_direction_prediction_network = CameraDirectionPredictor(nf, self.backbone_wrapper.backbone_wh, fea_output=3)
        self.attention = MultiHeadAttention(nf, nf + 14, nf, 1)
        self.hip_autograd = True
        self._packed = None
        self._packed_key = None
        self._key_cache = None
        self._key_cache_id = None
        self._key_cache_rays = None

    def _scorer_params(self):
        rp, at = self.ray_preprocessor, self.attention
        return {
            "ray_preprocessor.mlp.0.weight": rp.mlp[0].weight, "ray_preprocessor.mlp.0.bias": rp.mlp[0].bias,
            "ray_preprocessor.mlp.2.weight": rp.mlp[2].weight, "ray_preprocessor.mlp.2.bias": rp.mlp[2].bias,
            "ray_preprocessor.mlp2.0.weight": rp.mlp2[0].weight, "ray_preprocessor.mlp2.0.bias": rp.mlp2[0].bias,
            "ray_preprocessor.mlp2.2.weight": rp.mlp2[2].weight, "ray_preprocessor.mlp2.2.bias": rp.mlp2[2].bias,
            "attention.k_proj.weight": at.k_proj.weight, "attention.k_proj.bias": at.k_proj.bias,
            "attention.q_proj.weight": at.q_proj.weight, "attention.q_proj.bias": at.q_proj.bias,
        }

    def packed_weights(self, device) -> ops.PackedWeights:
        params = self._scorer_params()
        key = (str(device),) + tuple((p.data_ptr(), p._version) for p in params.values())
        if self._packed is None or self._packed_key != key:
            self._packed = ops.PackedWeights(params, device)
            self._packed_key = key
            self._key_cache = None
        return self._packed

    KEEP_FP32_KEYS_BELOW = 4_000_000

    def _ensure_keys(self, rays_ori, rays_dir, rays_rgb, profile=None, sample_min_rays: Optional[int] = None):
        w = self.packed_weights(rays_ori.device)
        mode = ops.effective_mma_mode()
        fmt = "f16-planes" if mode in ops.F16_MODES else f"f32-keys-mma{mode}"
        smin = ops.SELECT_MIN_RAYS if sample_min_rays is None else int(sample_min_rays)
        ident = (rays_ori.shape[0], rays_ori._version, rays_dir._version, rays_rgb._version, self._packed_key, fmt, rays_ori.shape[0] >= smin)
        held = self._key_cache_rays
        same = (self._key_cache is not None and self._key_cache_id == ident and held is not None
                and all(h is t or (h.data_ptr() == t.data_ptr() and h.shape == t.shape and h.stride() == t.stride())
                        for h, t in zip(held, (rays_ori, rays_dir, rays_rgb))))
        if not same:
            self._key_cache = self._key_cache_rays = None
            if ops.get_arena() is not None:
                self._select_ws = self._stream_sample = None
                ops.get_arena().reset(self)
            r = rays_ori.shape[0]
            planes_mode = mode in ops.F16_MODES
            keep_fp32 = (not planes_mode) or r <= self.KEEP_FP32_KEYS_BELOW
            scale = None
            norm = torch.zeros(1, device=rays_ori.device) if planes_mode else None
            if planes_mode:
                _, key, (planes, scale) = ops.ray_keys(rays_ori, rays_dir, rays_rgb, w, want_key=keep_fp32, profile=profile, want_planes=True, norm_out=norm)
            else:
                _, key = ops.ray_keys(rays_ori, rays_dir, rays_rgb, w, profile=profile)
                planes = None
            sample = None
            if planes_mode and r >= smin:
                si = ops.select_sample_indices(r, rays_ori.device)
                _, _, (s_planes, s_scale) = ops.ray_keys(rays_ori[si], rays_dir[si], rays_rgb[si], w, want_key=False, want_planes=True)
                sample = (s_planes, s_scale)
            self._key_cache, self._key_cache_id = {"key": key, "planes": planes, "scale": scale, "sample": sample, "norm": norm}, ident
            self._key_cache_rays = (rays_ori, rays_dir, rays_rgb)
        return self._key_cache

    def ray_keys(self, rays_ori, rays_dir, rays_rgb, profile=None) -> torch.Tensor:
        c = self._ensure_keys(rays_ori, rays_dir, rays_rgb, profile)
        if c["key"] is None:
            _, key = ops.ray_keys(rays_ori, rays_dir, rays_rgb, self.packed_weights(rays_ori.device))
            return key
        return c["key"]

    def ray_features(self, rays_ori, rays_dir, rays_rgb) -> torch.Tensor:
        feat, _ = ops.ray_keys(rays_ori, rays_dir, rays_rgb, self.packed_weights(rays_ori.device), want_feat=True, want_key=False)
        return feat

    def _full_ntok(self, b, device):
        c = getattr(self, "_ntok_cache", None)
        if c is None or c.shape[0] < b or c.device != device:
            self._ntok_cache = c = torch.full((max(b, 64),), ops.MAX_TOKENS, dtype=torch.int32, device=device)
        return c[:b]

    def _tokens_to_q(self, token_list, device):
        w = self.packed_weights(device)
        if isinstance(token_list, BatchedTokens):
            b, t = token_list.shape[0], token_list.shape[1]
            if t != ops.MAX_TOKENS:
                token_list = token_list.dense()
            else:
                wq, bq = self.attention.q_proj.weight, self.attention.q_proj.bias
                pe = token_list.pe
                c = getattr(self, "_peq", None)
                if c is None or c[0] != self._packed_key or c[1] is not pe or c[2] != pe._version:
                    self._peq = c = (self._packed_key, pe, pe._version, torch.addmm(bq.detach(), pe, wq.detach()[:, ops.D:].t()).contiguous(),
                                     wq.detach()[:, :ops.D].contiguous())
                q = ops.linear(token_list.feats.reshape(b * t, ops.D), c[4]).view(b, t, ops.D)
                q += c[3]
                return q, self._full_ntok(b, device), [t] * b
        if torch.is_tensor(token_list):
            tokens = token_list.contiguous()
            n_host = [tokens.shape[1]] * tokens.shape[0]
            n_tok = self._full_ntok(tokens.shape[0], tokens.device)
        else:
            tokens, n_tok = ops.pad_tokens(token_list, device)
            n_host = [int(t.shape[0]) for t in token_list]
        return ops.q_proj(tokens, n_tok, w), n_tok, n_host

    def invalidate_caches(self):
        self._packed = self._key_cache = self._key_cache_rays = self._select_ws = self._stream_sample = self._peq = None
        if ops.get_arena() is not None:
            ops.get_arena().reset(self)

    @torch.no_grad()
    def image_tokens_u8(self, imgs_u8: torch.Tensor, table256: torch.Tensor):
        bw = self.backbone_wrapper
        norm = bw.preprocess_batch_u8(imgs_u8, table256)
        if norm is None:
            return None
        return bw.assemble_batch(bw.features_from_norm(norm))

    @torch.no_grad()
    def image_tokens(self, imgs: Sequence[torch.Tensor], masks: Sequence[Optional[torch.Tensor]]):
        bw = self.backbone_wrapper
        if all(m is None for m in masks) and all(i.shape == imgs[0].shape for i in imgs):
            stacked = imgs if isinstance(imgs, torch.Tensor) and imgs.dim() == 4 else torch.stack(list(imgs))
            feats = bw.features_from_norm(bw.preprocess_batch(stacked))
            return bw.assemble_batch(feats)
        pre = [bw.preprocess(i, m) for i, m in zip(imgs, masks)]
        feats = bw.features_from_norm(torch.cat([p[0] for p in pre], dim=0))
        toks, fmaps = [], []
        for f, (_, mimg) in zip(feats, pre):
            t_pe, _, fmap = bw.assemble(f, mimg)
            toks.append(t_pe)
            fmaps.append(fmap)
        return toks, torch.stack(fmaps)

    @torch.no_grad()
    def camera_up(self, fmaps: torch.Tensor) -> torch.Tensor:
        up = self.camera_direction_prediction_network(fmaps)
        return torch.nn.functional.normalize(up, dim=-1)

    @torch.no_grad()
    def score_tokens(self, token_list: List[torch.Tensor], rays_ori, rays_dir, rays_rgb, rays_to_output: int = 100,
                     want_scores: bool = True, workspace: Optional[torch.Tensor] = None, images_in_flight: Optional[int] = None,
                     profile=None, defer_status: bool = False):
        rays_to_output = ops.check_topk(rays_to_output)
        kc = self._ensure_keys(rays_ori, rays_dir, rays_rgb)
        w = self.packed_weights(rays_ori.device)
        q, n_tok, n_host = self._tokens_to_q(token_list, rays_ori.device)
        self.last_scoring_path = "two-pass"
        self.pending_select = None
        capturing = torch.cuda.is_current_stream_capturing()
        if (not want_scores and kc.get("sample") is not None and ops.select_enabled() and ops.effective_mma_mode() in ops.F16_MODES
                and rays_to_output <= ops.SELECT_MAX_CANDIDATES and (defer_status or not capturing)):
            b, r = q.shape[0], rays_ori.shape[0]
            need = ops.score_select_workspace_bytes(r, b, rays_to_output, ops.SELECT_MAX_CANDIDATES)
            sw = getattr(self, "_select_ws", None)
            if sw is None or sw.numel() < need or sw.device != q.device:
                if capturing:
                    raise RuntimeError("6dgs_amd: the select workspace must exist before a hipGraph capture (run the batch once eagerly)")
                self._select_ws = sw = None
                self._select_ws = sw = ops.big_empty(need, torch.uint8, q.device)
            idx, val, status = ops.score_select(q, n_tok, kc["planes"], kc["scale"], kc["sample"][0], kc["sample"][1], rays_to_output,
                                                max_candidates=ops.SELECT_MAX_CANDIDATES, workspace=sw, profile=profile, n_tok_host=n_host,
                                                key_norm=kc["norm"])
            self.last_select_launches = ops.select_sweep_plan(n_host)
            self.last_scoring_path = "select"
            pend = dict(status=status, q=q, n_tok=n_tok, k=rays_to_output, workspace=workspace, images_in_flight=images_in_flight,
                        rays=(rays_ori, rays_dir, rays_rgb))
            if defer_status:
                self.pending_select = pend
                return idx, val, None
            idx, val, _ = self.finish_select(idx, val, pend)
            return idx, val, None
        idx, val, scores, _ = ops.score_topk(q, n_tok, kc["key"], rays_to_output, want_scores=want_scores, workspace=workspace,
                                             images_in_flight=images_in_flight, profile=profile, n_tok_host=n_host,
                                             key_planes=kc["planes"], key_scale=kc["scale"])
        return idx, val, scores

    @torch.no_grad()
    def finish_select(self, idx, val, pending=None, status_host=None):
        pend = pending if pending is not None else self.pending_select
        self.pending_select = None
        if pend is None:
            return idx, val, []
        st = pend["status"].tolist() if status_host is None else [int(v) for v in status_host]
        self.last_select_candidates = st
        redo = [i for i, v in enumerate(st) if v < 0]
        self.last_scoring_path = "select" if not redo else f"select+two-pass({len(redo)})"
        if redo:
            kc = self._ensure_keys(*pend["rays"])
            q, n_tok = pend["q"], pend["n_tok"]
            sel = torch.tensor(redo, device=q.device)
            i2, v2, _, _ = ops.score_topk(q[sel].contiguous(), n_tok[sel].contiguous(), kc["key"], pend["k"], want_scores=False,
                                          workspace=pend["workspace"], images_in_flight=pend["images_in_flight"], key_planes=kc["planes"],
                                          key_scale=kc["scale"])
            idx[sel], val[sel] = i2, v2
        return idx, val, redo

    @torch.no_grad()
    def score_tokens_ray_sharded(self, token_list, rays_ori, rays_dir, rays_rgb, ray_offset: int, r_total: int, rays_to_output: int = 100,
                                 group=None, profile=None, use_select: bool = True):
        from . import distributed as dd
        dev, k = rays_ori.device, ops.check_topk(rays_to_output)
        world = dd.world()
        kc = self._ensure_keys(rays_ori, rays_dir, rays_rgb, sample_min_rays=max(4096, ops.SELECT_MIN_RAYS // max(world, 1)))
        q, n_tok, n_host = self._tokens_to_q(token_list, dev)
        f16 = ops.effective_mma_mode() in ops.F16_MODES
        have = torch.tensor([1 if (kc.get("sample") is not None and f16 and use_select and ops.select_enabled()
                                  and k <= ops.SELECT_MAX_CANDIDATES) else 0,
                             0 if kc.get("sample") is None else int(kc["sample"][0].shape[0])], dtype=torch.int64, device=dev)
        if dd.is_dist():
            flag, cnt = have[:1].clone(), have[1:].clone()
            dd._all_reduce(flag, torch.distributed.ReduceOp.MIN, group)
            dd._all_reduce(cnt, torch.distributed.ReduceOp.SUM, group)
            have = torch.cat([flag, cnt])
        use, r_sample_total = bool(int(have[0])), int(have[1])
        b = q.shape[0]
        idx = torch.full((b, k), -1, dtype=torch.int64, device=dev)
        val = torch.full((b, k), float("nan"), device=dev)
        redo = list(range(b))
        self.last_scoring_path = f"ray-sharded x{world} two-pass"
        if use:
            idx, val, st = dd.score_select_ray_sharded(q, n_tok, kc["planes"], kc["scale"], kc["sample"][0], kc["sample"][1], ray_offset, r_total,
                                                       r_sample_total, k, n_tok_host=n_host, profile=profile, group=group, key_norm=kc["norm"])
            self.last_select_candidates = st
            redo = [i for i, v in enumerate(st) if v < 0]
            self.last_scoring_path = f"ray-sharded x{world} select" + (f"+two-pass({len(redo)})" if redo else "")
        if redo:
            sel = torch.tensor(redo, device=dev)
            i2, v2, _ = dd.score_topk_ray_sharded(q[sel].contiguous(), n_tok[sel].contiguous(), kc["key"], ray_offset, k, key_planes=kc["planes"],
                                                  key_scale=kc["scale"], group=group)
            idx[sel], val[sel] = i2, v2
        return idx, val

    @torch.no_grad()
    def score_tokens_streamed(self, token_list, rays_ori, rays_dir, rays_rgb, rays_to_output: int = 100, chunk_rays: int = 8_388_608,
                              profile=None, key_cache_bytes: Optional[int] = None, return_stats: bool = False, use_select: bool = True):
        rays_to_output = ops.check_topk(rays_to_output)
        dev = rays_ori.device
        w = self.packed_weights(dev)
        q, n_tok, n_host = self._tokens_to_q(token_list, dev)
        b, r, k = q.shape[0], rays_ori.shape[0], rays_to_output
        chunk = max(256, (min(chunk_rays, max(r, 1)) + 255) // 256 * 256)
        mode = ops.effective_mma_mode()
        f16 = planes_mode = mode in ops.F16_MODES
        self.last_scoring_path = "streamed two-pass"
        if (f16 and use_select and not return_stats and ops.select_enabled() and r >= ops.SELECT_MIN_RAYS and k <= ops.SELECT_MAX_CANDIDATES
                and not torch.cuda.is_current_stream_capturing()):
            cmax = ops.SELECT_MAX_CANDIDATES
            held = getattr(self, "_stream_sample", None)
            ident = (r, rays_ori._version, rays_dir._version, rays_rgb._version, self._packed_key)
            if not (held is not None and held[0] == ident and all(h.data_ptr() == t.data_ptr() for h, t in zip(held[1], (rays_ori, rays_dir, rays_rgb)))):
                self._stream_sample = held = None
                if ops.get_arena() is not None:
                    self._key_cache = self._key_cache_rays = self._select_ws = None
                    ops.get_arena().reset(self)
                si = ops.select_sample_indices(r, dev)
                _, _, (sp, sscale) = ops.ray_keys(rays_ori[si], rays_dir[si], rays_rgb[si], w, want_key=False, want_planes=True)
                self._stream_sample = held = (ident, (rays_ori, rays_dir, rays_rgb), sp, sscale)
            with ops.arena_scope():
                ss = ops.SelectStream(q, n_tok, r, k, cmax, n_host)
                ss.reserve(max(min(chunk, r), int(held[2].shape[0])))
                ss.begin(held[2], held[3])
                for r0 in range(0, r, chunk):
                    r1 = min(r0 + chunk, r)
                    with ops.arena_scope():
                        _, _, (planes, scale) = ops.ray_keys(rays_ori[r0:r1], rays_dir[r0:r1], rays_rgb[r0:r1], w, want_key=False, want_planes=True,
                                                             norm_out=ss.key_norm)
                        ss.sweep(planes, scale, r0, profile, update_norm=False)
                        del planes, scale
                cand, count = ss.candidates()
                inside = torch.arange(cmax, device=dev)[None, :] < count.clamp(min=0, max=cmax)[:, None]
                ci = torch.where(inside, cand, torch.zeros_like(cand)).reshape(-1)
                _, _, (cp, cs) = ops.ray_keys(rays_ori[ci], rays_dir[ci], rays_rgb[ci], w, want_key=False, want_planes=True)
                idx, val, status = ss.rescore(cp, cs, cand, count, compact=True)
            st = status.tolist()
            self.last_select_candidates = st
            redo = [i for i, v in enumerate(st) if v < 0]
            self.last_scoring_path = "streamed select" if not redo else f"streamed select+two-pass({len(redo)})"
            if redo:
                del ss
                sub = token_list[torch.tensor(redo, device=dev)] if (torch.is_tensor(token_list) or isinstance(token_list, BatchedTokens)) else [token_list[i] for i in redo]
                i2, v2 = self.score_tokens_streamed(sub, rays_ori, rays_dir, rays_rgb, k, chunk_rays, profile, key_cache_bytes, use_select=False)
                sel = torch.tensor(redo, device=dev)
                idx[sel], val[sel] = i2, v2
                self.last_scoring_path = f"streamed select+two-pass({len(redo)})"
            return idx, val
        with ops.arena_scope():
            ws = ops.big_empty(ops.score_topk_workspace_bytes(min(chunk, r), b, k, planes=planes_mode), torch.uint8, dev)
            n_c = min(chunk, r)
            per_ray = 1536 if f16 else 4 * ops.D
            if key_cache_bytes is None:
                transient = n_c * per_ray + int(_lib_ray_keys_ws(n_c, ops.RAY_KEYS_CHUNK_MIN if ops.get_arena() is not None else ops.RAY_KEYS_CHUNK))
                arena = ops.get_arena()
                from_arena = arena is not None and planes_mode and arena.buf.device == dev
                room = (arena.capacity - arena.mark()) if from_arena else torch.cuda.mem_get_info(dev)[0]
                key_cache_bytes = max(0, int(0.7 * (room - transient)))
            kept, kept_bytes = {}, 0

            def chunk_keys(r0):
                r1 = min(r0 + chunk, r)
                o, d, c = rays_ori[r0:r1], rays_dir[r0:r1], rays_rgb[r0:r1]
                if not planes_mode:
                    _, key = ops.ray_keys(o, d, c, w)
                    return (key, None, None)
                _, _, (planes, scale) = ops.ray_keys(o, d, c, w, want_key=False, want_planes=True)
                return (None, planes, scale)

            def chunk_pass1(r0, may_keep):
                nonlocal kept_bytes
                run = lambda ent: ops.score_pass1(q, n_tok, ent[0], ws, k, key_planes=ent[1], key_scale=ent[2], profile=profile, n_tok_host=n_host)
                if r0 in kept:
                    return run(kept.pop(r0))
                nbytes = (min(r0 + chunk, r) - r0) * per_ray
                if may_keep and kept_bytes + nbytes <= key_cache_bytes:
                    kept[r0], kept_bytes = chunk_keys(r0), kept_bytes + nbytes
                    return run(kept[r0])
                with ops.arena_scope():
                    return run(chunk_keys(r0))

            m_g = torch.full((b, ops.MAX_TOKENS), -float("inf"), device=dev)
            s_g = torch.zeros(b, ops.MAX_TOKENS, device=dev)
            for r0 in range(0, r, chunk):
                st = chunk_pass1(r0, True)
                m_c, s_c = st[..., 0], st[..., 1]
                m_n = torch.maximum(m_g, m_c)
                safe = torch.where(torch.isinf(m_n), torch.zeros_like(m_n), m_n)
                s_g = s_g * torch.exp(torch.where(torch.isinf(m_g), torch.full_like(m_g, -float("inf")), m_g - safe)) + \
                    s_c * torch.exp(torch.where(torch.isinf(m_c), torch.full_like(m_c, -float("inf")), m_c - safe))
                m_g = m_n
            glob = torch.stack([m_g, s_g], dim=-1).contiguous()
            best_i = torch.full((b, k), -1, dtype=torch.int64, device=dev)
            best_v = torch.full((b, k), float("nan"), device=dev)
            mass = torch.zeros(b, dtype=torch.float64, device=dev)
            from . import distributed as dd
            for r0 in range(0, r, chunk):
                chunk_pass1(r0, False)
                idx, val, sc = ops.score_pass2(glob, n_tok, min(r0 + chunk, r) - r0, ws, k, used_planes=planes_mode, want_scores=return_stats)
                if return_stats:
                    mass += sc.double().sum(dim=1)
                gi = torch.where(idx >= 0, idx + r0, idx)
                best_i, best_v = dd.merge_topk(torch.cat([best_i, gi], dim=1), torch.cat([best_v, val], dim=1), 0, k, group=False)
        if return_stats:
            return best_i, best_v, glob, mass
        return best_i, best_v

# ... 93 lines not shown
```

### 6dgs_amd/ops.py

```python
from __future__ import annotations

import ctypes as C
import functools
import math
import os
import threading
from typing import Optional, Tuple

import torch

from . import _lib
from ._lib import Profile, ScorerWeights, check

D = 384
MMA_DEFAULT, MMA_F32, MMA_BF16X6, MMA_F16X3, MMA_F16X3_L32 = -1, 0, 1, 2, 3
F16_MODES = (MMA_F16X3, MMA_F16X3_L32)
MMA_LIBRARY_DEFAULT = MMA_F16X3
_mma_mode = MMA_DEFAULT


def set_mma_mode(mode: int):
    global _mma_mode
    assert mode in (MMA_DEFAULT, MMA_F32, MMA_BF16X6, MMA_F16X3, MMA_F16X3_L32)
    _mma_mode = mode
# ... 1536 lines not shown
        n[i] = t.shape[0]
    return tok, n.to(device)


@_on_device
def q_proj(tokens: torch.Tensor, n_tok: torch.Tensor, weights: PackedWeights) -> torch.Tensor:
    tokens = _f32(tokens)
    _need_gpu(tokens, n_tok)
    b = tokens.shape[0]
    q = torch.empty(b, MAX_TOKENS, D, device=tokens.device)
    check(_lib.load().sixdgs_q_proj(_p(tokens), _p(n_tok), b, weights.ref, _p(q), _stream()), "q_proj")
    return q


def score_topk_workspace_bytes(r: int, batch: int, topk: int = 100, planes: bool = False) -> int:
    if planes:
        return int(_lib.load().sixdgs_score_topk_workspace_bytes_ex(int(r), int(batch), int(topk), effective_mma_mode(), 1))
    return int(_lib.load().sixdgs_score_topk_workspace_bytes(int(r), int(batch), int(topk)))


@_on_device
def score_topk(q: torch.Tensor, n_tok: torch.Tensor, key: Optional[torch.Tensor], topk: int = 100, want_scores: bool = True,
               want_stats: bool = False, workspace: Optional[torch.Tensor] = None, images_in_flight: Optional[int] = None,
               profile: Optional["KernelProfile"] = None, n_tok_host=None, key_planes: Optional[torch.Tensor] = None,
               key_scale: Optional[torch.Tensor] = None):
    q = _f32(q)
    key = _f32(key) if key is not None else None
    _need_gpu(q, key, n_tok, key_planes)
    lib = _lib.load()
    r = key.shape[0] if key is not None else key_planes.shape[0]
    b, dev = q.shape[0], q.device
    idx = torch.empty(b, topk, dtype=torch.int64, device=dev)
    val = torch.empty(b, topk, device=dev)
    scores = torch.empty(b, r, device=dev) if want_scores else None
    stats = torch.empty(b, MAX_TOKENS, 2, device=dev) if want_stats else None
    if workspace is None:
        inflight = b if images_in_flight is None else max(1, min(b, images_in_flight))
        workspace = torch.empty(score_topk_workspace_bytes(r, inflight, topk, planes=key_planes is not None), dtype=torch.uint8, device=dev)
    h_n = None
    if profile is not None and n_tok_host is not None:
        h_n = (C.c_int32 * b)(*[int(v) for v in n_tok_host])
    mode = effective_mma_mode()
    if key_planes is not None and mode in F16_MODES:
        if key_planes.shape[1] != 1536 or key_scale is None:
            raise RuntimeError("6dgs_amd: key planes are not in the format of the active MMA mode (scaled fp16 planes [R,1536] + key_scale)")
    elif key_planes is not None:
        if key is None:
            raise RuntimeError("6dgs_amd: MMA_F32 / MMA_BF16X6 score on fp32 keys: pass `key` (key planes are the operand of the fp16 x 3 kernels only)")
        key_planes = key_scale = None
    check(lib.sixdgs_score_topk_ex(_p(q), _p(n_tok), h_n, b, _p(key), _p(key_planes), _p(key_scale), r, int(topk), _p(scores), _p(idx), _p(val), _p(stats),
                                   _p(workspace), workspace.numel(), _stream(), profile.ref if profile is not None else None,
                                   _mma_mode), "score_topk")
    return idx, val, scores, stats


MAX_TOPK = 1024


def check_topk(k, what: str = "rays_to_output") -> int:
    if isinstance(k, bool) or int(k) != k or not 1 <= int(k) <= MAX_TOPK:
        raise ValueError(f"6dgs_amd: {what} = {k!r}: the top-k takes 1 <= k <= MAX_TOPK = {MAX_TOPK}")
    return int(k)


SELECT_MAX_CANDIDATES = 4096
SELECT_SAMPLE_STRIDE = 16
SELECT_SAMPLE_STRIDE_LARGE = 32
SELECT_LARGE_RAYS = 16_000_000
SELECT_SAMPLE_STRIDE_HUGE = 64
SELECT_HUGE_RAYS = 32_000_000
SELECT_MIN_RAYS = 1 << 20
_select_enabled = True


def set_select_enabled(on: bool):
    global _select_enabled
    _select_enabled = bool(on)


def select_enabled() -> bool:
    return _select_enabled


@_on_device
def select_sample_indices(r: int, device, stride: Optional[int] = None) -> torch.Tensor:
    if stride is None:
        stride = SELECT_SAMPLE_STRIDE_HUGE if r >= SELECT_HUGE_RAYS else (SELECT_SAMPLE_STRIDE_LARGE if r >= SELECT_LARGE_RAYS else SELECT_SAMPLE_STRIDE)
    n = r // stride
    i = torch.arange(n, dtype=torch.int64, device=device)
    return i * stride + (((i * 2654435761) & 0xFFFFFFFF) >> 13) % stride


@_on_device
def key_norm_max(planes: torch.Tensor, scale: torch.Tensor, out: Optional[torch.Tensor] = None) -> torch.Tensor:
    _need_gpu(planes, scale, out)
    if planes.shape[1] != 1536:
        raise RuntimeError("6dgs_amd: key_norm_max needs scaled fp16 key planes (MMA_F16X3)")
    if out is None:
        out = torch.zeros(1, device=planes.device)
    check(_lib.load().sixdgs_key_planes_norm_max(_p(planes), _p(scale), planes.shape[0], _p(out), _stream()), "key_planes_norm_max")
    return out


def score_select_workspace_bytes(r: int, batch: int, topk: int = 100, max_candidates: int = SELECT_MAX_CANDIDATES) -> int:
    return int(_lib.load().sixdgs_score_select_workspace_bytes(int(r), int(batch), int(topk), int(max_candidates)))


def select_sweep_plan(n_tok_host, batch: Optional[int] = None):
    lib = _lib.load()
    b = len(n_tok_host) if n_tok_host is not None else int(batch)
    h_n = (C.c_int32 * b)(*[int(v) for v in n_tok_host]) if n_tok_host is not None else None
    cap = max(1, b)
    slots, imgs = (C.c_int32 * cap)(), (C.c_int32 * cap)()
    n = lib.sixdgs_select_sweep_plan(h_n, b, slots, imgs, cap)
    if n < 0:
        check(n, "select_sweep_plan")
    return [(int(slots[i]), int(imgs[i])) for i in range(min(n, cap))]


@_on_device
def score_select(q: torch.Tensor, n_tok: torch.Tensor, key_planes: torch.Tensor, key_scale: torch.Tensor, sample_planes: torch.Tensor,
                 sample_scale: torch.Tensor, topk: int = 100, max_candidates: int = SELECT_MAX_CANDIDATES,
                 workspace: Optional[torch.Tensor] = None, profile: Optional["KernelProfile"] = None, n_tok_host=None,
                 key_norm: Optional[torch.Tensor] = None):
    q = _f32(q)
    _need_gpu(q, n_tok, key_planes, key_scale, sample_planes, sample_scale, key_norm)
    if key_norm is None:
        key_norm = key_norm_max(key_planes, key_scale)
    if key_planes.shape[1] != 1536 or sample_planes.shape[1] != 1536:
        raise RuntimeError("6dgs_amd: score_select needs scaled fp16 key planes (MMA_F16X3)")
    lib = _lib.load()
    b, dev, r, rs = q.shape[0], q.device, key_planes.shape[0], sample_planes.shape[0]
    idx = torch.empty(b, topk, dtype=torch.int64, device=dev)
    val = torch.empty(b, topk, device=dev)
    status = torch.empty(b, dtype=torch.int32, device=dev)
    if workspace is None:
        workspace = torch.empty(score_select_workspace_bytes(r, b, topk, max_candidates), dtype=torch.uint8, device=dev)
    h_n = (C.c_int32 * b)(*[int(v) for v in n_tok_host]) if n_tok_host is not None else None
    check(lib.sixdgs_score_select(_p(q), _p(n_tok), h_n, b, _p(key_planes), _p(key_scale), _p(key_norm), r, _p(sample_planes), _p(sample_scale), rs,
                                  int(topk), int(max_candidates), _p(idx), _p(val), _p(status), _p(workspace), workspace.numel(), _stream(),
                                  profile.ref if profile is not None else None), "score_select")
    return idx, val, status


class SelectStream:

    @_on_device
    def __init__(self, q: torch.Tensor, n_tok: torch.Tensor, r_total: int, topk: int = 100, max_candidates: int = SELECT_MAX_CANDIDATES,
                 n_tok_host=None):
        self.q, self.n_tok = _f32(q), n_tok
        _need_gpu(self.q, n_tok)
        self.b, self.dev = self.q.shape[0], self.q.device
        self.device = self.dev
        self.r, self.topk, self.cmax = int(r_total), int(topk), int(max_candidates)
        self.stride = (self.r + 255) // 256 * 256
        self.ctok = torch.empty(self.b, MAX_TOKENS, device=self.dev)
        self.gsum = torch.empty(self.b, MAX_TOKENS, device=self.dev)
        self.u = big_empty((self.b, self.stride), torch.float32, self.dev)
        self.utm = torch.empty(self.b, self.stride // 256, device=self.dev)
        self.key_norm = torch.zeros(1, device=self.dev)
        self.ws = torch.empty(1, dtype=torch.uint8, device=self.dev)
        self.h_n = (C.c_int32 * self.b)(*[int(v) for v in n_tok_host]) if n_tok_host is not None else None

    def _grow(self, need):
        if self.ws.numel() < need:
            self.ws = None
            self.ws = big_empty(need, torch.uint8, self.dev)

    def reserve(self, chunk_rows: int):
        lib = _lib.load()
        self._grow(max(lib.sixdgs_select_workspace_bytes(int(chunk_rows), self.b, self.topk, self.cmax),
                       lib.sixdgs_select_candidates_workspace_bytes(self.r, self.b, self.topk, self.cmax)))

    @_on_device
    def begin(self, sample_planes, sample_scale):
        _need_gpu(self.q, sample_planes, sample_scale)
        lib = _lib.load()
        self._grow(lib.sixdgs_select_workspace_bytes(sample_planes.shape[0], self.b, self.topk, self.cmax))
        check(lib.sixdgs_select_begin(_p(self.q), _p(self.n_tok), self.h_n, self.b, _p(sample_planes), _p(sample_scale), sample_planes.shape[0], self.r,
                                      _p(self.ctok), _p(self.gsum), _p(self.ws), self.ws.numel(), _stream()), "select_begin")

    @_on_device
    def sample_stats(self, sample_planes, sample_scale) -> torch.Tensor:
        _need_gpu(self.q, sample_planes, sample_scale)
        lib = _lib.load()
        self._grow(lib.sixdgs_select_workspace_bytes(sample_planes.shape[0], self.b, self.topk, self.cmax))
        stats = torch.empty(self.b, MAX_TOKENS, 2, device=self.dev)
        check(lib.sixdgs_select_sample_stats(_p(self.q), _p(self.n_tok), self.h_n, self.b, _p(sample_planes), _p(sample_scale), sample_planes.shape[0],
                                             _p(stats), _p(self.ws), self.ws.numel(), _stream()), "select_sample_stats")
        return stats

    @_on_device
    def prepare(self, stats: torch.Tensor, r_sample_total: int, r_total: int):
        stats = _f32(stats)
        _need_gpu(self.q, stats)
        check(_lib.load().sixdgs_select_prepare(_p(stats), _p(self.n_tok), self.b, int(r_sample_total), int(r_total), _p(self.ctok), _p(self.gsum),
                                                _stream()), "select_prepare")

    @_on_device
    def topk_u(self, exact: bool = False) -> torch.Tensor:
        lib = _lib.load()
        _need_gpu(self.q)
        self._grow(lib.sixdgs_select_candidates_workspace_bytes(self.r, self.b, self.topk, self.cmax))
        val = torch.empty(self.b, self.topk, device=self.dev)
        check(lib.sixdgs_select_topk_u(_p(self.u), self.stride, self.r, None if exact else _p(self.utm), self.b, self.topk, _p(val), _p(self.ws),
                                       self.ws.numel(), _stream()),
              "select_topk_u")
        return val

    @_on_device
    def sweep(self, planes, scale, ray_offset: int, profile: Optional["KernelProfile"] = None, update_norm: bool = True):
        if ray_offset % 256:
            raise RuntimeError("6dgs_amd: select sweep chunks must start at a multiple of 256 rays")
        _need_gpu(self.q, planes, scale)
        lib = _lib.load()
        rc = planes.shape[0]
        self._grow(lib.sixdgs_select_workspace_bytes(rc, self.b, self.topk, self.cmax))
        check(lib.sixdgs_select_sweep(_p(self.q), _p(self.n_tok), self.h_n, self.b, _p(planes), _p(scale), rc,
                                      _p(self.ctok), _p(self.gsum), C.c_void_p(self.u.data_ptr() + 4 * int(ray_offset)), self.stride,
                                      C.c_void_p(self.utm.data_ptr() + 4 * (int(ray_offset) // 256)),
                                      _p(self.ws), self.ws.numel(), _stream(), profile.ref if profile is not None else None), "select_sweep")
        if update_norm:
            key_norm_max(planes, scale, out=self.key_norm)

    @_on_device
    def candidates(self, uk: Optional[torch.Tensor] = None):
        lib = _lib.load()
        _need_gpu(self.q)
        self._grow(lib.sixdgs_select_candidates_workspace_bytes(self.r, self.b, self.topk, self.cmax))
        cand = torch.zeros(self.b, self.cmax, dtype=torch.int64, device=self.dev)
        count = torch.empty(self.b, dtype=torch.int32, device=self.dev)
        uk = _f32(uk) if uk is not None else None
        check(lib.sixdgs_select_candidates(_p(self.u), self.stride, self.r, _p(self.utm), _p(self.q), _p(self.n_tok), self.b, _p(self.gsum), _p(self.key_norm),
                                           _p(uk), self.topk, self.cmax, _p(cand), _p(count), _p(self.ws), self.ws.numel(), _stream()), "select_candidates")
        return cand, count

    @_on_device
    def rescore(self, planes, scale, cand, count, compact: bool, allow_fewer: bool = False):
        lib = _lib.load()
        _need_gpu(self.q, planes, scale, cand, count)
        idx = torch.empty(self.b, self.topk, dtype=torch.int64, device=self.dev)
        val = torch.empty(self.b, self.topk, device=self.dev)
        status = torch.empty(self.b, dtype=torch.int32, device=self.dev)
        self._grow(lib.sixdgs_select_candidates_workspace_bytes(self.r, self.b, self.topk, self.cmax))
        check(lib.sixdgs_select_rescore(_p(self.q), _p(self.n_tok), self.b, _p(planes), _p(scale), 1 if compact else 0, _p(self.ctok),
                                        _p(self.gsum), _p(cand), _p(count), self.r, self.topk, self.cmax, 1 if allow_fewer else 0, _p(idx), _p(val), _p(status),
                                        _p(self.ws), self.ws.numel(), _stream()), "select_rescore")
        return idx, val, status


@_on_device
def score_pass1(q: torch.Tensor, n_tok: torch.Tensor, key: Optional[torch.Tensor], workspace: torch.Tensor, topk: int = 100,
                key_planes: Optional[torch.Tensor] = None, key_scale: Optional[torch.Tensor] = None,
                profile: Optional["KernelProfile"] = None, n_tok_host=None) -> torch.Tensor:
    q = _f32(q)
    key = _f32(key) if key is not None else None
    _need_gpu(q, key, n_tok, key_planes, workspace)
    r = key.shape[0] if key is not None else key_planes.shape[0]
    b = q.shape[0]
    stats = torch.empty(b, MAX_TOKENS, 2, device=q.device)
    h_n = (C.c_int32 * b)(*[int(v) for v in n_tok_host]) if (profile is not None and n_tok_host is not None) else None
    check(_lib.load().sixdgs_score_pass1(_p(q), _p(n_tok), h_n, b, _p(key), _p(key_planes), _p(key_scale), r, int(topk), _p(stats),
                                         _p(workspace), workspace.numel(), _stream(), profile.ref if profile is not None else None,
                                         _mma_mode), "score_pass1")
    return stats


@_on_device
def score_pass2(stats: torch.Tensor, n_tok: torch.Tensor, r: int, workspace: torch.Tensor, topk: int = 100, used_planes: bool = True,
                want_scores: bool = True):
    stats = _f32(stats)
    _need_gpu(stats, n_tok, workspace)
# ... 196 lines not shown
```

### include/sixdgs.h

```cpp
#ifndef SIXDGS_H
#define SIXDGS_H

#include <stddef.h>
#include <stdint.h>

#ifdef __cplusplus
extern "C" {
#endif

#define SIXDGS_ABI_VERSION 10
#define SIXDGS_E_BADARG (-1)
#define SIXDGS_E_WORKSPACE (-2)
#define SIXDGS_E_UNSUPPORTED (-3)

#define SIXDGS_D 384
#define SIXDGS_RAY_IN 141
#define SIXDGS_RAY_IN_PAD 144
#define SIXDGS_HID 512
#define SIXDGS_TOK_IN 398
#define SIXDGS_MAX_TOKENS 256

typedef void* sixdgs_stream_t;

#define SIXDGS_MMA_DEFAULT (-1)
// ... 213 lines not shown
                  int relu, float* y, int64_t ldy, sixdgs_stream_t stream);
int sixdgs_linear_ex(const float* x, int64_t m, int k, int64_t ldx, const float* w, int64_t ldw, const float* b, int n,
                     int relu, float* y, int64_t ldy, sixdgs_stream_t stream, int mma_mode);
size_t sixdgs_linear_splitk_workspace_bytes(int64_t m, int n, int slices);
int sixdgs_linear_splitk(const float* x, int64_t m, int k, int64_t ldx, const float* w, int64_t ldw, const float* b, int n,
                         int relu, float* y, int64_t ldy, int slices, void* ws, size_t ws_bytes, sixdgs_stream_t stream,
                         int mma_mode);

#define SIXDGS_TOK_A_PLAIN 0
#define SIXDGS_TOK_A_LAYERNORM 1
#define SIXDGS_TOK_EPI_BIAS 0
#define SIXDGS_TOK_EPI_GELU 1
#define SIXDGS_TOK_EPI_RESID 2
size_t sixdgs_tok_pack_bytes(int n, int k);
int sixdgs_tok_pack(const float* w , int n, int k, int64_t ldw, void* planes, float* inv_scale , sixdgs_stream_t stream);
int sixdgs_tok_linear(const float* x, int64_t m, int k, int64_t ldx, int a_mode, const float* ln_weight, const float* ln_bias, float ln_eps,
                      const void* w_planes, const float* w_inv_scale, const float* bias , int n, int epilogue, const float* residual,
                      int64_t ldr, const float* gamma, float* y, int64_t ldy, sixdgs_stream_t stream);

int sixdgs_tok_attention(const float* qkv, int64_t ldq, int images, int tokens, int heads, float* y, int64_t ldy, sixdgs_stream_t stream);

int sixdgs_im2col(const float* x, int64_t stride_b, int64_t stride_c, int64_t stride_y, int64_t stride_x, int batch, int channels, int height, int width, int k,
                  int taps_major, float* a, sixdgs_stream_t stream);

int sixdgs_u8_to_planar(const uint8_t* images, int batch, int64_t pixels, const float* table256, float* out, sixdgs_stream_t stream);

int sixdgs_image_prep(const uint8_t* images, int batch, int height, int width, const float* table256, int resized_h, int resized_w, int crop_top, int crop_left,
                      int out_size, const float* mean3, const float* std3, float* out, sixdgs_stream_t stream);

int sixdgs_q_proj(const float* tokens, const int32_t* d_n_tok, int batch,
                  const sixdgs_scorer_weights* w, float* q, sixdgs_stream_t stream);

size_t sixdgs_score_topk_workspace_bytes(int64_t r, int batch, int topk);
size_t sixdgs_score_topk_workspace_bytes_ex(int64_t r, int batch, int topk, int mma_mode, int with_key_planes);
int sixdgs_score_topk(const float* q , const int32_t* d_n_tok, int batch, const float* key ,
                      int64_t r, int topk, float* scores , int64_t* idx ,
                      float* val , float* row_stats , void* ws,
                      size_t ws_bytes, sixdgs_stream_t stream);
int sixdgs_score_topk_ex(const float* q, const int32_t* d_n_tok, const int32_t* h_n_tok ,
                         int batch, const float* key, const void* key_planes, const float* d_key_scale, int64_t r, int topk,
                         float* scores, int64_t* idx, float* val, float* row_stats, void* ws, size_t ws_bytes,
                         sixdgs_stream_t stream, sixdgs_profile* prof, int mma_mode);

int sixdgs_score_pass1(const float* q, const int32_t* d_n_tok, const int32_t* h_n_tok, int batch, const float* key,
                       const void* key_planes, const float* d_key_scale, int64_t r, int topk, float* row_stats, void* ws,
                       size_t ws_bytes, sixdgs_stream_t stream, sixdgs_profile* prof, int mma_mode);
int sixdgs_score_pass2(const float* row_stats, const int32_t* d_n_tok, int batch, int used_planes, int64_t r, int topk,
                       float* scores, int64_t* idx, float* val, void* ws, size_t ws_bytes, sixdgs_stream_t stream, int mma_mode);
size_t sixdgs_score_backward_workspace_bytes(int batch);
int sixdgs_score_backward(const float* q, const int32_t* d_n_tok, int batch, const float* key , int64_t r,
                          const float* row_stats, const float* g, float* dq, float* dk, void* ws, size_t ws_bytes, sixdgs_stream_t stream);
size_t sixdgs_score_backward_split_workspace_bytes(int batch, int64_t r, int ray_groups);
int sixdgs_score_backward_split(const float* q, const int32_t* d_n_tok, int batch, const float* key , int64_t r,
                                const float* row_stats, const float* g, float* dq, float* dk, int ray_groups, void* ws, size_t ws_bytes,
                                sixdgs_stream_t stream);
size_t sixdgs_score_select_workspace_bytes(int64_t r, int batch, int topk, int max_candidates);
int sixdgs_key_planes_norm_max(const void* planes, const float* d_scale, int64_t rows, float* d_norm_max, sixdgs_stream_t stream);
size_t sixdgs_select_workspace_bytes(int64_t r, int batch, int topk, int max_candidates);
size_t sixdgs_select_candidates_workspace_bytes(int64_t r, int batch, int topk, int max_candidates);
int sixdgs_select_sweep_plan(const int32_t* h_n_tok, int batch, int32_t* slots_per_launch, int32_t* images_per_launch, int max_launches);
int sixdgs_select_begin(const float* q, const int32_t* d_n_tok, const int32_t* h_n_tok, int batch, const void* sample_planes, const float* d_sample_scale,
                        int64_t r_sample, int64_t r_total, float* ctok, float* gsum, void* ws, size_t ws_bytes, sixdgs_stream_t stream);
int sixdgs_select_sample_stats(const float* q, const int32_t* d_n_tok, const int32_t* h_n_tok, int batch, const void* sample_planes, const float* d_sample_scale,
                               int64_t r_sample, float* row_stats , void* ws, size_t ws_bytes, sixdgs_stream_t stream);
int sixdgs_select_prepare(const float* row_stats, const int32_t* d_n_tok, int batch, int64_t r_sample, int64_t r_total, float* ctok, float* gsum,
                          sixdgs_stream_t stream);
int sixdgs_select_topk_u(const float* u, int64_t u_stride, int64_t r, const float* u_tile_max , int batch, int topk, float* val ,
                         void* ws, size_t ws_bytes, sixdgs_stream_t stream);
int sixdgs_select_sweep(const float* q, const int32_t* d_n_tok, const int32_t* h_n_tok, int batch, const void* key_planes,
                        const float* d_key_scale, int64_t r, const float* ctok, float* gsum, float* u, int64_t u_stride, float* u_tile_max,
                        void* ws, size_t ws_bytes, sixdgs_stream_t stream, sixdgs_profile* prof);
int sixdgs_select_candidates(const float* u, int64_t u_stride, int64_t r, const float* u_tile_max , const float* q, const int32_t* d_n_tok, int batch, const float* gsum,
                             const float* d_key_norm_max, const float* d_uk ,
                             int topk, int max_candidates, int64_t* cand, int32_t* d_count, void* ws, size_t ws_bytes, sixdgs_stream_t stream);
int sixdgs_select_rescore(const float* q, const int32_t* d_n_tok, int batch, const void* planes, const float* d_scale, int compact,
                          const float* ctok, const float* gsum, const int64_t* cand, const int32_t* d_count, int64_t r, int topk,
                          int max_candidates, int allow_fewer, int64_t* idx, float* val, int32_t* d_status, void* ws, size_t ws_bytes,
                          sixdgs_stream_t stream);
int sixdgs_score_select(const float* q, const int32_t* d_n_tok, const int32_t* h_n_tok ,
                        int batch, const void* key_planes, const float* d_key_scale, const float* d_key_norm_max, int64_t r,
                        const void* sample_planes, const float* d_sample_scale, int64_t r_sample, int topk, int max_candidates, int64_t* idx ,
                        float* val , int32_t* d_status , void* ws, size_t ws_bytes, sixdgs_stream_t stream,
                        sixdgs_profile* prof);
size_t sixdgs_topk_workspace_bytes(int64_t r, int batch, int topk);
int sixdgs_topk(const float* scores, int64_t r, int batch, int topk, int64_t* idx, float* val, void* ws,
                size_t ws_bytes, sixdgs_stream_t stream);

size_t sixdgs_distance_target_workspace_bytes(int64_t r);
int sixdgs_distance_target(const float* rays_ori, const float* rays_dir, int64_t r, const float* d_pose, int n_tokens,
                           float* target , float* d_sum, void* ws, size_t ws_bytes, sixdgs_stream_t stream);

int sixdgs_solve_pose(const float* rays_ori, const float* rays_dir, int64_t r, const int64_t* idx ,
                      const float* val , int k, const float* up , const float* gt_c2w ,
                      int batch, float* c2w, int32_t* status, float* w_final, int32_t* n_kept, float* centre ,
                      float* errors, sixdgs_stream_t stream);

size_t sixdgs_solve_pose_consensus_workspace_bytes(int batch, int k);
int sixdgs_solve_pose_consensus(const float* rays_ori, const float* rays_dir, int64_t r, const int64_t* idx ,
                                const float* val , int k, const float* up , const float* gt_c2w ,
                                int batch, float tau, int prior, float* c2w, int32_t* status, float* w_final, int32_t* n_kept,
                                float* centre , float* errors, float* support, int32_t* n_inliers, float* rms,
                                int32_t* winner, void* ws, size_t ws_bytes, sixdgs_stream_t stream);

#ifdef __cplusplus
}
#endif
#endif
```

Baseline: 75.64.

## Add f16 high-pair sample plane layout and dedicated prepass kernel for selection

```diff
diff --git a/6dgs_amd/_lib.py b/6dgs_amd/_lib.py
--- a/6dgs_amd/_lib.py
+++ b/6dgs_amd/_lib.py
@@ -111,6 +111,10 @@
     "sixdgs_select_rescore": (i32, [vp, vp, i32, vp, vp, i32, vp, vp, vp, vp, i64, i32, i32, i32, vp, vp, vp, vp, sz, vp]),
     "sixdgs_select_sample_stats": (i32, [vp, vp, vp, i32, vp, vp, i64, vp, vp, sz, vp]),
     "sixdgs_select_prepare": (i32, [vp, vp, i32, i64, i64, vp, vp, vp]),
+    "sixdgs_planes_to_h_pairs": (i32, [vp, i64, vp, vp]),
+    "sixdgs_select_sample_stats_h": (i32, [vp, vp, vp, i32, vp, vp, vp, i64, vp, vp, sz, vp]),
+    "sixdgs_select_begin_h": (i32, [vp, vp, vp, i32, vp, vp, vp, i64, i64, vp, vp, vp, sz, vp]),
+    "sixdgs_score_select_h": (i32, [vp, vp, vp, i32, vp, vp, vp, i64, vp, vp, vp, i64, i32, i32, vp, vp, vp, vp, sz, vp, C.POINTER(Profile)]),
     "sixdgs_select_topk_u": (i32, [vp, i64, i64, vp, i32, i32, vp, vp, sz, vp]),
     "sixdgs_linear_splitk_workspace_bytes": (sz, [i64, i32, i32]),
     "sixdgs_linear_splitk": (i32, [vp, i64, i32, i64, vp, i64, vp, i32, i32, vp, i64, i32, vp, sz, vp, i32]),
diff --git a/6dgs_amd/build.py b/6dgs_amd/build.py
--- a/6dgs_amd/build.py
+++ b/6dgs_amd/build.py
@@ -9,7 +9,7 @@
 LIB = os.path.join(CSRC, "lib6dgs_hip.so")
 HOSTCHECK = os.path.join(CSRC, "libsixdgs_hostcheck.so")
 SOURCES = ["geometry.hip", "gemm.hip", "dense.hip", "score.hip", "score_bwd.hip", "pose.hip", "pose_consensus.hip", "vit.hip", "splat.hip", "raster.hip", "photometric.hip", "refine.hip", "fit.hip", "densify.hip", "knn.hip", "pyramid.hip"]
-HEADERS = ["common.h", "device_math.h", "gemm_kernel.h", "dense.h", os.path.join("..", "..", "include", "sixdgs.h"), "dense_layout.h", "sweep_plan.h", "sweep_layout.h", "pose_step.h", "adam_step.h", "render_pass.h", "densify_rules.h", "knn_rules.h", "pyramid_rules.h"]
+HEADERS = ["common.h", "device_math.h", "gemm_kernel.h", "dense.h", os.path.join("..", "..", "include", "sixdgs.h"), "dense_layout.h", "sweep_plan.h", "sweep_layout.h", "prepass_layout.h", "pose_step.h", "adam_step.h", "render_pass.h", "densify_rules.h", "knn_rules.h", "pyramid_rules.h"]
 HIPCC = os.environ.get("HIPCC", "/opt/rocm/bin/hipcc")
 FLAGS = ["--offload-arch=gfx950", "-O3", "-std=c++17", "-fPIC", "-ffp-contract=off", "-Wall", "-Wno-unused-function"]
 FLAGS += os.environ.get("SIXDGS_EXTRA_FLAGS", "").split()
@@ -49,7 +49,7 @@
 def build_hostcheck(force: bool = False) -> str:
     src = os.path.join(CSRC, "hostcheck.cpp")
     deps = [src, os.path.join(CSRC, "device_math.h"), os.path.join(CSRC, "dense_layout.h"), os.path.join(CSRC, "sweep_plan.h"),
-            os.path.join(CSRC, "sweep_layout.h"), os.path.join(CSRC, "pose_step.h"), os.path.join(CSRC, "adam_step.h"), os.path.join(CSRC, "densify_rules.h"),
+            os.path.join(CSRC, "sweep_layout.h"), os.path.join(CSRC, "prepass_layout.h"), os.path.join(CSRC, "pose_step.h"), os.path.join(CSRC, "adam_step.h"), os.path.join(CSRC, "densify_rules.h"),
             os.path.join(CSRC, "knn_rules.h"), os.path.join(CSRC, "pyramid_rules.h")]
     if force or _stale(HOSTCHECK, deps):
         cmd = [HIPCC, "-x", "hip", "--offload-arch=gfx950", "-O2", "-std=c++17", "-fPIC", "-ffp-contract=off", "-shared", src,
diff --git a/6dgs_amd/csrc/hostcheck.cpp b/6dgs_amd/csrc/hostcheck.cpp
--- a/6dgs_amd/csrc/hostcheck.cpp
+++ b/6dgs_amd/csrc/hostcheck.cpp
@@ -4,6 +4,7 @@
 #include "sweep_plan.h"
 #include "dense_layout.h"
 #include "sweep_layout.h"
+#include "prepass_layout.h"
 #include "pose_step.h"
 #include "adam_step.h"
 #include "densify_rules.h"
@@ -337,6 +338,19 @@
 void hc_pyr_keep_input(const float* best_loss_last, const float* loss_input, long long n, int* keep) {
   for (long long i = 0; i < n; ++i) keep[i] = pyr::keep_input(best_loss_last[i], loss_input[i]) ? 1 : 0;
 }
+int hc_hp_const(int which) {
+  const int v[] = {hp::kSrcRowBytes, hp::kRowBytes, hp::kStages, hp::kStageBytes, hp::kSlabs};
+  return which >= 0 && which < 5 ? v[which] : -1;
+}
+int hc_hp_src_offset(int slab, int plane, int c) { return hp::src_offset(slab, plane, c); }
+int hc_hp_pair_offset(int slab, int c) { return hp::pair_offset(slab, c); }
+int hc_hp_piece_row(int piece, int lane) { return hp::piece_row(piece, lane); }
+unsigned hc_hp_piece_src_offset(int piece, int lane, int stage) { return hp::piece_src_offset(piece, lane, stage); }
+unsigned hc_hp_piece_lds_offset(int piece, int lane) { return hp::piece_lds_offset(piece, lane); }
+unsigned hc_hp_frag_offset(int row0, int lane, int ks, int par) { return hp::frag_offset(row0, lane, ks, par); }
+int hc_hp_frag_k(int stage, int par, int ks, int lane, int e) { return hp::frag_k(stage, par, ks, lane, e); }
+int hc_hp_kstep_order(int stage, int par, int ks) { return hp::kstep_order(stage, par, ks); }
+
 int hc_dl_const(int which) {
   const int v[] = {dl::kSlabB, dl::kPRow, dl::kGran, dl::kGranSlab, dl::kChunkRun};
   return which >= 0 && which < 5 ? v[which] : -1;
diff --git a/6dgs_amd/csrc/prepass_layout.h b/6dgs_amd/csrc/prepass_layout.h
--- /dev/null
+++ b/6dgs_amd/csrc/prepass_layout.h
@@ -0,0 +1,29 @@
+#pragma once
+#include <hip/hip_runtime.h>
+
+namespace sdg {
+namespace hp {
+
+#define SDG_HP __host__ __device__ __forceinline__ constexpr
+
+constexpr int kSrcRowBytes = 1536, kRowBytes = 768, kStages = 6, kStageBytes = 128, kSlabs = 12;
+
+SDG_HP int src_offset(int slab, int plane, int c) { return slab * 128 + plane * 64 + c * 16; }
+SDG_HP int pair_offset(int slab, int c) { return (slab >> 1) * kStageBytes + (slab & 1) * 64 + c * 16; }
+
+SDG_HP int piece_row(int piece, int lane) { return 8 * piece + (lane >> 3); }
+SDG_HP int piece_src_chunk(int piece, int lane) { return (lane & 7) ^ ((piece_row(piece, lane) >> 1) & 7); }
+SDG_HP unsigned piece_src_offset(int piece, int lane, int stage) { return (unsigned)(stage * kStageBytes + (piece_src_chunk(piece, lane) << 4)); }
+SDG_HP unsigned piece_lds_offset(int piece, int lane) { return (unsigned)(1024 * piece + 16 * lane); }
+
+SDG_HP int frag_chunk(int lane, int ks, int par) { return par * 4 + 2 * ks + (lane >> 5); }
+SDG_HP unsigned frag_offset(int row0, int lane, int ks, int par) {
+  const int row = row0 + (lane & 31);
+  return (unsigned)(row * 128 + ((frag_chunk(lane, ks, par) ^ ((row >> 1) & 7)) << 4));
+}
+SDG_HP int frag_k(int stage, int par, int ks, int lane, int e) { return 32 * (2 * stage + par) + 16 * ks + 8 * (lane >> 5) + e; }
+SDG_HP int kstep_order(int stage, int par, int ks) { return 2 * (2 * stage + par) + ks; }
+
+#undef SDG_HP
+}
+}
diff --git a/6dgs_amd/csrc/score.hip b/6dgs_amd/csrc/score.hip
--- a/6dgs_amd/csrc/score.hip
+++ b/6dgs_amd/csrc/score.hip
@@ -5,6 +5,7 @@
 #include "gemm_kernel.h"
 #include "sweep_plan.h"
 #include "sweep_layout.h"
+#include "prepass_layout.h"
 
 using namespace sdg;
 
@@ -859,6 +860,271 @@
   } while (PERS && (grp += A.n_sets) < A.n_groups);
 }
 
+template <bool PERS>
+__global__ void __launch_bounds__(512, 1) k_prepass_h(LogitsF16Args A) {
+  constexpr int kRowH = hp::kRowBytes, kStage = 2 * kQStageX;
+  __shared__ __attribute__((aligned(1024))) char lds[kLdsX];
+  const unsigned w = xcd_remap(blockIdx.x, gridDim.x);
+  const int bl = (int)(w % (unsigned)A.nb);
+  const int set = (int)(w / (unsigned)A.nb);
+  const int b = A.b0 + bl;
+  const int M = A.n_tok[b];
+  const int tid = threadIdx.x, lane = tid & 63;
+  const int wave = __builtin_amdgcn_readfirstlane(tid >> 6);
+  const int wm = wave >> 1, wn = wave & 1;
+  const float cq = A.q_quarter_scales ? A.qinv[4 * b + wm] : A.qinv[2 * b + (wm >> 1)];
+  const bool active = wm * 64 < M;
+  const int t_base = A.n_tiles / A.n_groups, t_rem = A.n_tiles - t_base * A.n_groups;
+  const int n_tiles128 = (int)((A.r + 127) >> 7);
+  int grp = set;
+  do {
+  float* pout = A.partial + ((int64_t)bl * A.n_groups + grp) * kT * 2;
+  float m_run[2] = {-INFINITY, -INFINITY}, s_run[2] = {0.f, 0.f};
+  const int t_begin = grp * t_base + min(grp, t_rem);
+  const int t_end = t_begin + t_base + (grp < t_rem ? 1 : 0);
+  if (M > 0 && t_begin < t_end) {
+    const unsigned lds0 = (unsigned)(uintptr_t)(lds_ptr_t)lds;
+    int lane_p = lane;
+    if (PERS) asm volatile("" : "+v"(lane_p));
+    unsigned offQ[4], offK[4];
+    int rowK[4];
+#pragma unroll
+    for (int i = 0; i < 4; ++i) {
+      const int piece = wave * 4 + i, row = hp::piece_row(piece, lane_p);
+      const unsigned inrow = (unsigned)(hp::piece_src_chunk(piece, lane_p) << 4);
+      offQ[i] = (unsigned)min(row, M - 1) * kRowH + inrow;
+      offK[i] = inrow;
+      rowK[i] = row;
+    }
+    const char* qbase = A.qp + (int64_t)b * kT * kRowH;
+    auto issue_q = [&](const int s, const int qstage, const int i) {
+      __builtin_amdgcn_global_load_lds((gbl_ptr_t)(qbase + (offQ[i] + (unsigned)(s * hp::kStageBytes))),
+                                       (lds_ptr_t)(lds + qstage * kStage + (wave * 4 + i) * 1024), 16, 0, 0);
+    };
+    auto issue_k = [&](const char* kbase, int lim, const int s, const int kstage, const int i) {
+      const unsigned ob = (unsigned)min(rowK[i], lim) * kRowH + offK[i] + (unsigned)(s * hp::kStageBytes);
+      __builtin_amdgcn_global_load_lds((gbl_ptr_t)(kbase + ob), (lds_ptr_t)(lds + kKBaseX + kstage * kStage + (wave * 4 + i) * 1024), 16, 0, 2);
+    };
+    auto tile_lim = [&](int tile) {
+      const int64_t left = A.r - (int64_t)tile * kBNX - 1;
+      return left < kBNX - 1 ? (int)left : kBNX - 1;
+    };
+    unsigned fa[2][2], fb[2][2], fb2[2][2];
+#pragma unroll
+    for (int ks = 0; ks < 2; ++ks)
+#pragma unroll
+      for (int par = 0; par < 2; ++par) {
+        fa[ks][par] = lds0 + hp::frag_offset(wm * 64, lane_p, ks, par);
+        fb[ks][par] = lds0 + kKBaseX + hp::frag_offset(wn * 128, lane_p, ks, par);
+        fb2[ks][par] = fb[ks][par] + 65536u;
+      }
+    auto read_a = [&](const int t, const int ks, const int par, const int qstage) { return lds_read_frag_h_off(fa[ks][par], qstage * kStage + t * 4096); };
+    auto read_b = [&](const int t, const int ks, const int par, const int kstage) {
+      const int off = kstage * kStage + t * 4096;
+      return off < 65536 ? lds_read_frag_h_off(fb[ks][par], off & 65535) : lds_read_frag_h_off(fb2[ks][par], off & 65535);
+    };
+    const char* kcur = A.kp + (int64_t)t_begin * kBNX * kRowH;
+    int lim_cur = tile_lim(t_begin);
+
+    f16x8 a0[2], a1[2], b0[2], b1[2];
+    auto wait_lds = [&]() {
+      asm volatile("s_waitcnt lgkmcnt(0)" ::: "memory");
+      __builtin_amdgcn_sched_barrier(0);
+    };
+#pragma unroll
+    for (int i = 0; i < 4; ++i) issue_k(kcur, lim_cur, 0, 0, i);
+#pragma unroll
+    for (int i = 0; i < 4; ++i) issue_q(0, 0, i);
+#pragma unroll
+    for (int i = 0; i < 4; ++i) issue_k(kcur, lim_cur, 1, 1, i);
+#pragma unroll
+    for (int i = 0; i < 4; ++i) issue_q(1, 1, i);
+#pragma unroll
+    for (int i = 0; i < 4; ++i) issue_k(kcur, lim_cur, 2, 2, i);
+    asm volatile("s_waitcnt vmcnt(12)" ::: "memory");
+    __builtin_amdgcn_s_barrier();
+#pragma unroll
+    for (int t = 0; t < 2; ++t) {
+      a0[t] = read_a(t, 0, 0, 0);
+      b0[t] = read_b(t, 0, 0, 0);
+    }
+    wait_lds();
+
+    for (int tile = t_begin; tile < t_end; ++tile) {
+      const bool has_next = tile + 1 < t_end;
+      const char* knext = has_next ? kcur + (int64_t)kBNX * kRowH : kcur;
+      const int lim_next = has_next ? tile_lim(tile + 1) : lim_cur;
+      asm volatile("" : "+v"(offQ[0]), "+v"(offQ[1]), "+v"(offQ[2]), "+v"(offQ[3]), "+v"(offK[0]), "+v"(offK[1]), "+v"(offK[2]), "+v"(offK[3]));
+      if (!active) {
+        int ks3 = 0;
+#pragma unroll 1
+        for (int j = 0; j < hp::kStages; ++j) {
+          asm volatile("s_waitcnt vmcnt(4)" ::: "memory");
+          __builtin_amdgcn_s_barrier();
+          const int sq = j + 2 < hp::kStages ? j + 2 : j + 2 - hp::kStages;
+#pragma unroll
+          for (int i = 0; i < 4; ++i) issue_q(sq, j & 1, i);
+          const bool nxt = j + 3 >= hp::kStages;
+          const char* kb = nxt ? knext : kcur;
+          const int kl = nxt ? lim_next : lim_cur, sk = nxt ? j + 3 - hp::kStages : j + 3;
+#pragma unroll
+          for (int i = 0; i < 4; ++i) issue_k(kb, kl, sk, ks3, i);
+          ks3 = ks3 == 2 ? 0 : ks3 + 1;
+        }
+        kcur = knext;
+        lim_cur = lim_next;
+        continue;
+      }
+      f32x16 acc[2][4];
+#pragma unroll
+      for (int i = 0; i < 2; ++i)
+#pragma unroll
+        for (int j = 0; j < 4; ++j)
+#pragma unroll
+          for (int r = 0; r < 16; ++r) acc[i][j][r] = 0.f;
+
+      auto mfma_step = [&](f16x8 (&xa)[2], f16x8 (&xb)[2], const int h, auto side) {
+        side();
+        __builtin_amdgcn_sched_barrier(0);
+#pragma unroll
+        for (int z = 0; z < 4; ++z) {
+          const int tm = z >> 1, tn = z & 1;
+          acc[tm][2 * h + tn] = __builtin_amdgcn_mfma_f32_32x32x16_f16(xb[tn], xa[tm], acc[tm][2 * h + tn], 0, 0, 0);
+          __builtin_amdgcn_sched_barrier(0);
+        }
+        wait_lds();
+      };
+#pragma unroll
+      for (int j = 0; j < hp::kStages; ++j) {
+        const int qs = j & 1, ks3 = j % 3;
+        const int qn = (j + 1) & 1, kn = (j + 1) % 3;
+#pragma unroll
+        for (int par = 0; par < 2; ++par) {
+          mfma_step(a0, b0, 0, [&]() {
+            b1[0] = read_b(2, 0, par, ks3);
+            b1[1] = read_b(3, 0, par, ks3);
+          });
+          mfma_step(a0, b1, 1, [&]() {
+            a1[0] = read_a(0, 1, par, qs);
+            a1[1] = read_a(1, 1, par, qs);
+            b0[0] = read_b(0, 1, par, ks3);
+            b0[1] = read_b(1, 1, par, ks3);
+          });
+          mfma_step(a1, b0, 0, [&]() {
+            b1[0] = read_b(2, 1, par, ks3);
+            b1[1] = read_b(3, 1, par, ks3);
+          });
+          if (par == 0) {
+            mfma_step(a1, b1, 1, [&]() {
+              a0[0] = read_a(0, 0, 1, qs);
+              a0[1] = read_a(1, 0, 1, qs);
+              b0[0] = read_b(0, 0, 1, ks3);
+              b0[1] = read_b(1, 0, 1, ks3);
+            });
+          } else {
+            asm volatile("s_waitcnt vmcnt(4)" ::: "memory");
+            __builtin_amdgcn_s_barrier();
+            mfma_step(a1, b1, 1, [&]() {
+              a0[0] = read_a(0, 0, 0, qn);
+              a0[1] = read_a(1, 0, 0, qn);
+              b0[0] = read_b(0, 0, 0, kn);
+              b0[1] = read_b(1, 0, 0, kn);
+#pragma unroll
+              for (int i = 0; i < 4; ++i) issue_q((j + 2) % hp::kStages, qs, i);
+#pragma unroll
+              for (int i = 0; i < 4; ++i) {
+                if (j + 3 < hp::kStages) issue_k(kcur, lim_cur, j + 3, ks3, i);
+                else issue_k(knext, lim_next, j + 3 - hp::kStages, ks3, i);
+              }
+            });
+          }
+        }
+      }
+
+      {
+        const int t128 = min(2 * tile + wn, n_tiles128 - 1);
+        const float cf = (cq * load_uniform(A.kinv + t128)) * kInvSqrtD;
+        const bool ragged = lim_cur < kBNX - 1;
+#pragma unroll
+        for (int tm = 0; tm < 2; ++tm) {
+          float mx = -INFINITY;
+#pragma unroll
+          for (int tn = 0; tn < 4; ++tn)
+#pragma unroll
+            for (int rg = 0; rg < 4; ++rg) {
+              float4 v;
+              v.x = acc[tm][tn][4 * rg + 0] * cf;
+              v.y = acc[tm][tn][4 * rg + 1] * cf;
+              v.z = acc[tm][tn][4 * rg + 2] * cf;
+              v.w = acc[tm][tn][4 * rg + 3] * cf;
+              acc[tm][tn][4 * rg + 0] = v.x;
+              acc[tm][tn][4 * rg + 1] = v.y;
+              acc[tm][tn][4 * rg + 2] = v.z;
+              acc[tm][tn][4 * rg + 3] = v.w;
+              mx = fmaxf(mx, fmaxf(fmaxf(v.x, v.y), fmaxf(v.z, v.w)));
+            }
+          const float mn = fmaxf(m_run[tm], mx);
+          float sum[4] = {0.f, 0.f, 0.f, 0.f};
+          if (!ragged) {
+#pragma unroll
+            for (int tn = 0; tn < 4; ++tn)
+#pragma unroll
+              for (int r = 0; r < 16; ++r) sum[r & 3] += __expf(acc[tm][tn][r] - mn);
+          } else {
+            int ray0 = wn * 128 + 4 * (lane >> 5);
+            asm volatile("" : "+v"(ray0));
+#pragma unroll
+            for (int tn = 0; tn < 4; ++tn)
+#pragma unroll
+              for (int r = 0; r < 16; ++r)
+                sum[r & 3] += (ray0 + tn * 32 + 8 * (r >> 2) + (r & 3) <= lim_cur) ? __expf(acc[tm][tn][r] - mn) : 0.f;
+          }
+          s_run[tm] = s_run[tm] * __expf(m_run[tm] - mn) + ((sum[0] + sum[1]) + (sum[2] + sum[3]));
+          m_run[tm] = mn;
+        }
+      }
+      kcur = knext;
+      lim_cur = lim_next;
+    }
+    asm volatile("s_waitcnt vmcnt(0)" ::: "memory");
+  }
+  __syncthreads();
+  float(*part)[256][2] = reinterpret_cast<float(*)[256][2]>(lds);
+#pragma unroll
+  for (int tm = 0; tm < 2; ++tm) {
+    float* pp = part[wn * 2 + (lane >> 5)][wm * 64 + tm * 32 + (lane & 31)];
+    pp[0] = m_run[tm];
+    pp[1] = s_run[tm];
+  }
+  __syncthreads();
+  if (tid < 256) {
+    float m = -INFINITY, sres = 0.f;
+#pragma unroll
+    for (int h = 0; h < 4; ++h) {
+      const float mt = part[h][tid][0], st2 = part[h][tid][1];
+      if (mt > -INFINITY) {
+        const float mn = fmaxf(m, mt);
+        sres = sres * __expf(m - mn) + st2 * __expf(mt - mn);
+        m = mn;
+      }
+    }
+    pout[2 * tid] = m;
+    pout[2 * tid + 1] = sres;
+  }
+  if (PERS) __syncthreads();
+  } while (PERS && (grp += A.n_sets) < A.n_groups);
+}
+
+__global__ void __launch_bounds__(256) k_hpairs_from_planes(const char* __restrict__ src, int64_t rows, char* __restrict__ dst) {
+  const int64_t n = rows * 48;
+  for (int64_t i = (int64_t)blockIdx.x * 256 + threadIdx.x; i < n; i += (int64_t)gridDim.x * 256) {
+    const int64_t row = i / 48;
+    const int k8 = (int)(i - row * 48);
+    *reinterpret_cast<f16x8*>(dst + row * hp::kRowBytes + hp::pair_offset(k8 >> 2, k8 & 3)) =
+        *reinterpret_cast<const f16x8*>(src + row * hp::kSrcRowBytes + hp::src_offset(k8 >> 2, 0, k8 & 3));
+  }
+}
+
 __global__ void __launch_bounds__(256) k_split_tiles_f16(const float* __restrict__ src, int64_t rows, int64_t ld, char* __restrict__ dst,
                                                          float* __restrict__ inv_scale) {
   __shared__ float wmax[4];
@@ -1291,7 +1557,7 @@
 
 __global__ void __launch_bounds__(256) k_split_q_slots(const float* __restrict__ q, const int* __restrict__ n_tok, const SweepSlots T, char* __restrict__ dst,
                                                        float* __restrict__ inv_scale, const float* __restrict__ ctok, float* __restrict__ ctok_slot,
-                                                       int* __restrict__ slot_rows) {
+                                                       int* __restrict__ slot_rows, const int h_pairs = 0) {
   __shared__ float wmax[4];
   const int slot = blockIdx.x >> 2, w = blockIdx.x & 3;
   const int img = T.q_img[slot][w], lq = T.q_lq[slot][w];
@@ -1315,7 +1581,7 @@
   }
   const float sc = ldexpf(1.f, sh);
   if (threadIdx.x == 0) inv_scale[blockIdx.x] = ldexpf(1.f, -sh);
-  char* const drow = dst + ((int64_t)slot * kT + 64 * w) * kRowF;
+  char* const drow = dst + ((int64_t)slot * kT + 64 * w) * (h_pairs ? hp::kRowBytes : kRowF);
   for (int i = threadIdx.x; i < 64 * 48; i += 256) {
     const int row = i / 48, k8 = i - row * 48;
     f16x8 h, l;
@@ -1333,6 +1599,10 @@
     } else {
 #pragma unroll
       for (int e = 0; e < 8; ++e) h[e] = l[e] = (_Float16)0.f;
+    }
+    if (h_pairs) {
+      *reinterpret_cast<f16x8*>(drow + (int64_t)row * hp::kRowBytes + hp::pair_offset(k8 >> 2, k8 & 3)) = h;
+      continue;
     }
     char* d = drow + (int64_t)row * kRowF + (k8 >> 2) * kSlabF + (k8 & 3) * 16;
     *reinterpret_cast<f16x8*>(d) = h;
@@ -2251,21 +2521,38 @@
   return (int)plan.size();
 }
 
+int sixdgs_planes_to_h_pairs(const void* planes, int64_t rows, void* h_pairs, sixdgs_stream_t stream) {
+  SDG_CHECK_ARG(rows >= 0);
+  if (rows == 0) return 0;
+  SDG_CHECK_ARG(planes && h_pairs && ((uintptr_t)planes % 16) == 0 && ((uintptr_t)h_pairs % 16) == 0);
+  const int64_t blocks = sdg_cdiv(rows * 48, 256);
+  hipLaunchKernelGGL(k_hpairs_from_planes, dim3((unsigned)(blocks < 16384 ? blocks : 16384)), dim3(256), 0, sdg_stream(stream), (const char*)planes, rows,
+                     (char*)h_pairs);
+  SDG_LAUNCH_OK();
+  return 0;
+}
+
 int sixdgs_select_sample_stats(const float* q, const int32_t* d_n_tok, const int32_t* h_n_tok, int batch, const void* sample_planes,
                                const float* d_sample_scale, int64_t r_sample, float* row_stats, void* ws, size_t ws_bytes, sixdgs_stream_t stream) {
+  return sixdgs_select_sample_stats_h(q, d_n_tok, h_n_tok, batch, sample_planes, nullptr, d_sample_scale, r_sample, row_stats, ws, ws_bytes, stream);
+}
+
+int sixdgs_select_sample_stats_h(const float* q, const int32_t* d_n_tok, const int32_t* h_n_tok, int batch, const void* sample_planes, const void* sample_h,
+                                 const float* d_sample_scale, int64_t r_sample, float* row_stats, void* ws, size_t ws_bytes, sixdgs_stream_t stream) {
   SDG_CHECK_ARG(batch >= 0 && batch <= 32767 && r_sample >= 1);
   if (batch == 0) return 0;
   SDG_CHECK_ARG(q && d_n_tok && sample_planes && d_sample_scale && row_stats && ws && ((uintptr_t)sample_planes % 16) == 0 &&
-                ((uintptr_t)q % 16) == 0 && ((uintptr_t)ws % 256) == 0);
+                ((uintptr_t)sample_h % 16) == 0 && ((uintptr_t)q % 16) == 0 && ((uintptr_t)ws % 256) == 0);
   hipStream_t s = sdg_stream(stream);
   SelectWs w;
   if (!select_ws(ws, ws_bytes, r_sample, batch, 1, 8, &w)) return SIXDGS_E_WORKSPACE;
   const int n_groups = f16x_groups(r_sample);
   for (const SweepSlots& T : sweep_pack(h_n_tok, batch, sweep_slot_cap())) {
     if (T.n_slots > 0) {
+      const bool h_pairs = sample_h != nullptr && prepass_one_term(T.n_slots);
       hipLaunchKernelGGL(k_split_q_slots, dim3((unsigned)(4 * T.n_slots)), dim3(256), 0, s, q, d_n_tok, T, w.qplanes, w.qinv, (const float*)nullptr,
-                         (float*)nullptr, w.slot_rows);
-      LogitsF16Args V = select_args(w.slot_rows, T.n_slots, w, sample_planes, d_sample_scale, r_sample);
+                         (float*)nullptr, w.slot_rows, h_pairs ? 1 : 0);
+      LogitsF16Args V = select_args(w.slot_rows, T.n_slots, w, h_pairs ? sample_h : sample_planes, d_sample_scale, r_sample);
       V.q_quarter_scales = 1;
       static const int reserve_env = [] { const char* e = getenv("SIXDGS_PREPASS_RESERVE_CUS"); return e ? atoi(e) : -2; }();
       const int reserve = reserve_env != -2 ? reserve_env : (T.n_slots == 1 ? kPrepassReserveCusOneSlot : kPrepassReserveCus);
@@ -2275,10 +2562,12 @@
         V.sib_sync = nullptr;
         V.sib_extra = 0u;
         V.sib_period = kSibPeriod;
-        if (prepass_one_term(T.n_slots)) hipLaunchKernelGGL((k_logits_f16x<kOneTerm, kOutStats, true>), dim3((unsigned)(V.n_sets * T.n_slots)), dim3(512), 0, s, V);
+        if (h_pairs) hipLaunchKernelGGL((k_prepass_h<true>), dim3((unsigned)(V.n_sets * T.n_slots)), dim3(512), 0, s, V);
+        else if (prepass_one_term(T.n_slots)) hipLaunchKernelGGL((k_logits_f16x<kOneTerm, kOutStats, true>), dim3((unsigned)(V.n_sets * T.n_slots)), dim3(512), 0, s, V);
         else hipLaunchKernelGGL((k_logits_f16x<kAllTerms, kOutStats, true>), dim3((unsigned)(V.n_sets * T.n_slots)), dim3(512), 0, s, V);
       } else {
-        if (prepass_one_term(T.n_slots)) hipLaunchKernelGGL((k_logits_f16x<kOneTerm, kOutStats>), dim3((unsigned)(V.n_groups * T.n_slots)), dim3(512), 0, s, V);
+        if (h_pairs) hipLaunchKernelGGL((k_prepass_h<false>), dim3((unsigned)(V.n_groups * T.n_slots)), dim3(512), 0, s, V);
+        else if (prepass_one_term(T.n_slots)) hipLaunchKernelGGL((k_logits_f16x<kOneTerm, kOutStats>), dim3((unsigned)(V.n_groups * T.n_slots)), dim3(512), 0, s, V);
         else hipLaunchKernelGGL((k_logits_f16x<kAllTerms, kOutStats>), dim3((unsigned)(V.n_groups * T.n_slots)), dim3(512), 0, s, V);
       }
     }
@@ -2303,12 +2592,18 @@
 
 int sixdgs_select_begin(const float* q, const int32_t* d_n_tok, const int32_t* h_n_tok, int batch, const void* sample_planes, const float* d_sample_scale,
                         int64_t r_sample, int64_t r_total, float* ctok, float* gsum, void* ws, size_t ws_bytes, sixdgs_stream_t stream) {
+  return sixdgs_select_begin_h(q, d_n_tok, h_n_tok, batch, sample_planes, nullptr, d_sample_scale, r_sample, r_total, ctok, gsum, ws, ws_bytes, stream);
+}
+
+int sixdgs_select_begin_h(const float* q, const int32_t* d_n_tok, const int32_t* h_n_tok, int batch, const void* sample_planes, const void* sample_h,
+                          const float* d_sample_scale, int64_t r_sample, int64_t r_total, float* ctok, float* gsum, void* ws, size_t ws_bytes,
+                          sixdgs_stream_t stream) {
   SDG_CHECK_ARG(batch >= 0 && r_sample >= 1 && r_total >= r_sample);
   if (batch == 0) return 0;
   SDG_CHECK_ARG(ws && ((uintptr_t)ws % 256) == 0);
   SelectWs w;
   if (!select_ws(ws, ws_bytes, r_sample, batch, 1, 8, &w)) return SIXDGS_E_WORKSPACE;
-  const int st = sixdgs_select_sample_stats(q, d_n_tok, h_n_tok, batch, sample_planes, d_sample_scale, r_sample, w.stats, ws, ws_bytes, stream);
+  const int st = sixdgs_select_sample_stats_h(q, d_n_tok, h_n_tok, batch, sample_planes, sample_h, d_sample_scale, r_sample, w.stats, ws, ws_bytes, stream);
   if (st) return st;
   return sixdgs_select_prepare(w.stats, d_n_tok, batch, r_sample, r_total, ctok, gsum, stream);
 }
@@ -2462,6 +2757,14 @@
                         const float* d_key_scale, const float* d_key_norm_max, int64_t r, const void* sample_planes, const float* d_sample_scale,
                         int64_t r_sample, int topk, int max_candidates, int64_t* idx, float* val, int32_t* d_status, void* ws, size_t ws_bytes,
                         sixdgs_stream_t stream, sixdgs_profile* prof) {
+  return sixdgs_score_select_h(q, d_n_tok, h_n_tok, batch, key_planes, d_key_scale, d_key_norm_max, r, sample_planes, nullptr, d_sample_scale, r_sample, topk,
+                               max_candidates, idx, val, d_status, ws, ws_bytes, stream, prof);
+}
+
+int sixdgs_score_select_h(const float* q, const int32_t* d_n_tok, const int32_t* h_n_tok, int batch, const void* key_planes,
+                          const float* d_key_scale, const float* d_key_norm_max, int64_t r, const void* sample_planes, const void* sample_h,
+                          const float* d_sample_scale, int64_t r_sample, int topk, int max_candidates, int64_t* idx, float* val, int32_t* d_status, void* ws,
+                          size_t ws_bytes, sixdgs_stream_t stream, sixdgs_profile* prof) {
   SDG_CHECK_ARG(r >= 1 && r_sample >= 1 && r_sample <= r && batch >= 0 && topk >= 1 && topk <= 1024 && max_candidates >= topk &&
                 max_candidates <= (1 << 20) && (max_candidates % 8) == 0);
   if (batch == 0) return 0;
@@ -2483,7 +2786,7 @@
     const int nb = (int)((batch - b0) < bg ? (batch - b0) : bg);
     const float* qg = q + (int64_t)b0 * kT * SIXDGS_D;
     const int32_t* ng = d_n_tok + b0;
-    int st = sixdgs_select_begin(qg, ng, h_n_tok ? h_n_tok + b0 : nullptr, nb, sample_planes, d_sample_scale, r_sample, r, ctok, gsum, ws, stage, stream);
+    int st = sixdgs_select_begin_h(qg, ng, h_n_tok ? h_n_tok + b0 : nullptr, nb, sample_planes, sample_h, d_sample_scale, r_sample, r, ctok, gsum, ws, stage, stream);
     if (st) return st;
     st = sixdgs_select_sweep(qg, ng, h_n_tok ? h_n_tok + b0 : nullptr, nb, key_planes, d_key_scale, r, ctok, gsum, u, (int64_t)stride, utm, ws, stage,
                              stream, prof);
diff --git a/6dgs_amd/distributed.py b/6dgs_amd/distributed.py
--- a/6dgs_amd/distributed.py
+++ b/6dgs_amd/distributed.py
@@ -358,14 +358,15 @@
 
 def score_select_ray_sharded(q: torch.Tensor, n_tok: torch.Tensor, key_planes: torch.Tensor, key_scale: torch.Tensor, sample_planes: torch.Tensor,
                              sample_scale: torch.Tensor, ray_offset: int, r_total: int, r_sample_total: int, topk: int = 100,
-                             max_candidates: Optional[int] = None, n_tok_host=None, profile=None, group=None, key_norm: Optional[torch.Tensor] = None):
+                             max_candidates: Optional[int] = None, n_tok_host=None, profile=None, group=None, key_norm: Optional[torch.Tensor] = None,
+                             sample_h: Optional[torch.Tensor] = None):
     from . import ops
 
     r_local = key_planes.shape[0]
     cmax = ops.SELECT_MAX_CANDIDATES if max_candidates is None else int(max_candidates)
     with ops.arena_scope():
         ss = ops.SelectStream(q, n_tok, r_local, topk, cmax, n_tok_host)
-        stats = merge_row_stats(ss.sample_stats(sample_planes, sample_scale), group)
+        stats = merge_row_stats(ss.sample_stats(sample_planes, sample_scale, sample_h), group)
         ss.prepare(stats, r_sample_total, r_total)
         if key_norm is not None:
             ss.key_norm.copy_(key_norm)
diff --git a/6dgs_amd/identification_module.py b/6dgs_amd/identification_module.py
--- a/6dgs_amd/identification_module.py
+++ b/6dgs_amd/identification_module.py
@@ -124,7 +124,7 @@
             if planes_mode and r >= smin:
                 si = ops.select_sample_indices(r, rays_ori.device)
                 _, _, (s_planes, s_scale) = ops.ray_keys(rays_ori[si], rays_dir[si], rays_rgb[si], w, want_key=False, want_planes=True)
-                sample = (s_planes, s_scale)
+                sample = (s_planes, s_scale, ops.sample_h_pairs(s_planes))
             self._key_cache, self._key_cache_id = {"key": key, "planes": planes, "scale": scale, "sample": sample, "norm": norm}, ident
             self._key_cache_rays = (rays_ori, rays_dir, rays_rgb)
         return self._key_cache
@@ -228,7 +228,7 @@
                 self._select_ws = sw = ops.big_empty(need, torch.uint8, q.device)
             idx, val, status = ops.score_select(q, n_tok, kc["planes"], kc["scale"], kc["sample"][0], kc["sample"][1], rays_to_output,
                                                 max_candidates=ops.SELECT_MAX_CANDIDATES, workspace=sw, profile=profile, n_tok_host=n_host,
-                                                key_norm=kc["norm"])
+                                                key_norm=kc["norm"], sample_h=kc["sample"][2])
             self.last_select_launches = ops.select_sweep_plan(n_host)
             self.last_scoring_path = "select"
             pend = dict(status=status, q=q, n_tok=n_tok, k=rays_to_output, workspace=workspace, images_in_flight=images_in_flight,
@@ -288,7 +288,8 @@
         self.last_scoring_path = f"ray-sharded x{world} two-pass"
         if use:
             idx, val, st = dd.score_select_ray_sharded(q, n_tok, kc["planes"], kc["scale"], kc["sample"][0], kc["sample"][1], ray_offset, r_total,
-                                                       r_sample_total, k, n_tok_host=n_host, profile=profile, group=group, key_norm=kc["norm"])
+                                                       r_sample_total, k, n_tok_host=n_host, profile=profile, group=group, key_norm=kc["norm"],
+                                                       sample_h=kc["sample"][2])
             self.last_select_candidates = st
             redo = [i for i, v in enumerate(st) if v < 0]
             self.last_scoring_path = f"ray-sharded x{world} select" + (f"+two-pass({len(redo)})" if redo else "")
@@ -323,11 +324,11 @@
                     ops.get_arena().reset(self)
                 si = ops.select_sample_indices(r, dev)
                 _, _, (sp, sscale) = ops.ray_keys(rays_ori[si], rays_dir[si], rays_rgb[si], w, want_key=False, want_planes=True)
-                self._stream_sample = held = (ident, (rays_ori, rays_dir, rays_rgb), sp, sscale)
+                self._stream_sample = held = (ident, (rays_ori, rays_dir, rays_rgb), sp, sscale, ops.sample_h_pairs(sp))
             with ops.arena_scope():
                 ss = ops.SelectStream(q, n_tok, r, k, cmax, n_host)
                 ss.reserve(max(min(chunk, r), int(held[2].shape[0])))
-                ss.begin(held[2], held[3])
+                ss.begin(held[2], held[3], held[4])
                 for r0 in range(0, r, chunk):
                     r1 = min(r0 + chunk, r)
                     with ops.arena_scope():
diff --git a/6dgs_amd/ops.py b/6dgs_amd/ops.py
--- a/6dgs_amd/ops.py
+++ b/6dgs_amd/ops.py
@@ -1642,6 +1642,36 @@
     return _select_enabled
 
 
+_prepass_h_pairs = os.environ.get("SIXDGS_PREPASS_H_PAIRS", "1") != "0"
+
+
+def set_prepass_h_pairs(on: bool):
+    global _prepass_h_pairs
+    _prepass_h_pairs = bool(on)
+
+
+def prepass_h_pairs() -> bool:
+    return _prepass_h_pairs
+
+
+@_on_device
+def sample_h_pairs(sample_planes: torch.Tensor) -> torch.Tensor:
+    _need_gpu(sample_planes)
+    if sample_planes.dim() != 2 or sample_planes.shape[1] != 1536 or not sample_planes.is_contiguous():
+        raise RuntimeError("6dgs_amd: sample_h_pairs needs contiguous scaled fp16 planes [rows, 1536] (MMA_F16X3)")
+    out = torch.empty(sample_planes.shape[0], 768, dtype=torch.uint8, device=sample_planes.device)
+    check(_lib.load().sixdgs_planes_to_h_pairs(_p(sample_planes), sample_planes.shape[0], _p(out), _stream()), "planes_to_h_pairs")
+    return out
+
+
+def _sample_h(sample_planes, sample_h):
+    if sample_h is None or not _prepass_h_pairs:
+        return None
+    if sample_h.dtype != torch.uint8 or tuple(sample_h.shape) != (sample_planes.shape[0], 768) or not sample_h.is_contiguous():
+        raise RuntimeError("6dgs_amd: sample_h must be sample_h_pairs(sample_planes): uint8 [rows, 768]")
+    return sample_h
+
+
 @_on_device
 def select_sample_indices(r: int, device, stride: Optional[int] = None) -> torch.Tensor:
     if stride is None:
@@ -1682,9 +1712,9 @@
 def score_select(q: torch.Tensor, n_tok: torch.Tensor, key_planes: torch.Tensor, key_scale: torch.Tensor, sample_planes: torch.Tensor,
                  sample_scale: torch.Tensor, topk: int = 100, max_candidates: int = SELECT_MAX_CANDIDATES,
                  workspace: Optional[torch.Tensor] = None, profile: Optional["KernelProfile"] = None, n_tok_host=None,
-                 key_norm: Optional[torch.Tensor] = None):
+                 key_norm: Optional[torch.Tensor] = None, sample_h: Optional[torch.Tensor] = None):
     q = _f32(q)
-    _need_gpu(q, n_tok, key_planes, key_scale, sample_planes, sample_scale, key_norm)
+    _need_gpu(q, n_tok, key_planes, key_scale, sample_planes, sample_scale, key_norm, sample_h)
     if key_norm is None:
         key_norm = key_norm_max(key_planes, key_scale)
     if key_planes.shape[1] != 1536 or sample_planes.shape[1] != 1536:
@@ -1697,9 +1727,10 @@
     if workspace is None:
         workspace = torch.empty(score_select_workspace_bytes(r, b, topk, max_candidates), dtype=torch.uint8, device=dev)
     h_n = (C.c_int32 * b)(*[int(v) for v in n_tok_host]) if n_tok_host is not None else None
-    check(lib.sixdgs_score_select(_p(q), _p(n_tok), h_n, b, _p(key_planes), _p(key_scale), _p(key_norm), r, _p(sample_planes), _p(sample_scale), rs,
-                                  int(topk), int(max_candidates), _p(idx), _p(val), _p(status), _p(workspace), workspace.numel(), _stream(),
-                                  profile.ref if profile is not None else None), "score_select")
+    check(lib.sixdgs_score_select_h(_p(q), _p(n_tok), h_n, b, _p(key_planes), _p(key_scale), _p(key_norm), r, _p(sample_planes),
+                                    _p(_sample_h(sample_planes, sample_h)), _p(sample_scale), rs,
+                                    int(topk), int(max_candidates), _p(idx), _p(val), _p(status), _p(workspace), workspace.numel(), _stream(),
+                                    profile.ref if profile is not None else None), "score_select")
     return idx, val, status
 
 
@@ -1733,21 +1764,23 @@
                        lib.sixdgs_select_candidates_workspace_bytes(self.r, self.b, self.topk, self.cmax)))
 
     @_on_device
-    def begin(self, sample_planes, sample_scale):
-        _need_gpu(self.q, sample_planes, sample_scale)
+    def begin(self, sample_planes, sample_scale, sample_h=None):
+        _need_gpu(self.q, sample_planes, sample_scale, sample_h)
         lib = _lib.load()
         self._grow(lib.sixdgs_select_workspace_bytes(sample_planes.shape[0], self.b, self.topk, self.cmax))
-        check(lib.sixdgs_select_begin(_p(self.q), _p(self.n_tok), self.h_n, self.b, _p(sample_planes), _p(sample_scale), sample_planes.shape[0], self.r,
-                                      _p(self.ctok), _p(self.gsum), _p(self.ws), self.ws.numel(), _stream()), "select_begin")
+        check(lib.sixdgs_select_begin_h(_p(self.q), _p(self.n_tok), self.h_n, self.b, _p(sample_planes), _p(_sample_h(sample_planes, sample_h)),
+                                        _p(sample_scale), sample_planes.shape[0], self.r,
+                                        _p(self.ctok), _p(self.gsum), _p(self.ws), self.ws.numel(), _stream()), "select_begin")
 
     @_on_device
-    def sample_stats(self, sample_planes, sample_scale) -> torch.Tensor:
-        _need_gpu(self.q, sample_planes, sample_scale)
+    def sample_stats(self, sample_planes, sample_scale, sample_h=None) -> torch.Tensor:
+        _need_gpu(self.q, sample_planes, sample_scale, sample_h)
         lib = _lib.load()
         self._grow(lib.sixdgs_select_workspace_bytes(sample_planes.shape[0], self.b, self.topk, self.cmax))
         stats = torch.empty(self.b, MAX_TOKENS, 2, device=self.dev)
-        check(lib.sixdgs_select_sample_stats(_p(self.q), _p(self.n_tok), self.h_n, self.b, _p(sample_planes), _p(sample_scale), sample_planes.shape[0],
-                                             _p(stats), _p(self.ws), self.ws.numel(), _stream()), "select_sample_stats")
+        check(lib.sixdgs_select_sample_stats_h(_p(self.q), _p(self.n_tok), self.h_n, self.b, _p(sample_planes), _p(_sample_h(sample_planes, sample_h)),
+                                               _p(sample_scale), sample_planes.shape[0],
+                                               _p(stats), _p(self.ws), self.ws.numel(), _stream()), "select_sample_stats")
         return stats
 
     @_on_device
diff --git a/include/sixdgs.h b/include/sixdgs.h
--- a/include/sixdgs.h
+++ b/include/sixdgs.h
@@ -319,6 +319,17 @@
                         const void* sample_planes, const float* d_sample_scale, int64_t r_sample, int topk, int max_candidates, int64_t* idx ,
                         float* val , int32_t* d_status , void* ws, size_t ws_bytes, sixdgs_stream_t stream,
                         sixdgs_profile* prof);
+int sixdgs_planes_to_h_pairs(const void* planes, int64_t rows, void* h_pairs, sixdgs_stream_t stream);
+int sixdgs_select_sample_stats_h(const float* q, const int32_t* d_n_tok, const int32_t* h_n_tok, int batch, const void* sample_planes, const void* sample_h,
+                                 const float* d_sample_scale, int64_t r_sample, float* row_stats , void* ws, size_t ws_bytes,
+                                 sixdgs_stream_t stream);
+int sixdgs_select_begin_h(const float* q, const int32_t* d_n_tok, const int32_t* h_n_tok, int batch, const void* sample_planes, const void* sample_h,
+                          const float* d_sample_scale, int64_t r_sample, int64_t r_total, float* ctok, float* gsum, void* ws, size_t ws_bytes,
+                          sixdgs_stream_t stream);
+int sixdgs_score_select_h(const float* q, const int32_t* d_n_tok, const int32_t* h_n_tok, int batch, const void* key_planes, const float* d_key_scale,
+                          const float* d_key_norm_max, int64_t r, const void* sample_planes, const void* sample_h, const float* d_sample_scale,
+                          int64_t r_sample, int topk, int max_candidates, int64_t* idx, float* val, int32_t* d_status, void* ws, size_t ws_bytes,
+                          sixdgs_stream_t stream, sixdgs_profile* prof);
 size_t sixdgs_topk_workspace_bytes(int64_t r, int batch, int topk);
 int sixdgs_topk(const float* scores, int64_t r, int batch, int topk, int64_t* idx, float* val, void* ws,
                 size_t ws_bytes, sixdgs_stream_t stream);
```

Result: no change. 75.77 (median of 6 runs) (+0.2%).
